# tnwei/waternet

Measured on NVIDIA H100. Metric: images/sec at 1080p batch16 (preprocess + gated-fusion forward, uint8 in -> uint8 out), higher is better.
Workload: dtype bf16 + fp8 corrections (v = hi + lo: hi x hi in bf16, both correction terms of the heavy layers as one e4m3 MMA; fp32 accumulate; 3-term bf16 elsewhere)

## Files before the change

### waternet_b200/csrc/common.cuh

```cuda
#pragma once

#include <cuda_runtime.h>
#include <stdint.h>
#include <stdio.h>

#include "../../include/waternet_b200.h"
#include "tiling.cuh"

namespace wn {

void set_error(const char* fmt, ...);

inline size_t align256(size_t v) { return (v + 255) / 256 * 256; }

#define WN_CUDA(call)                                                                   \
  do {                                                                                  \
    cudaError_t err__ = (call);                                                         \
    if (err__ != cudaSuccess) {                                                         \
      wn::set_error("%s:%d: %s -> %s", __FILE__, __LINE__, #call, cudaGetErrorString(err__)); \
      return WN_E_CUDA;                                                                 \
    }                                                                                   \
  } while (0)

#define WN_LAUNCH_CHECK(h)   \
  do {                       \
    (h)->launches++;         \
    WN_CUDA(cudaGetLastError()); \
  } while (0)

struct Tables {
  uint16_t gtab[256];
  uint16_t ctab[3072];
  int16_t ytab[256];
  int16_t fytab[256];
  uint8_t igtab[4096];
  uint8_t gamma[256];
  float div255[256];
};

void build_tables_host(Tables* t);

struct LayerDesc {
  int cin, cout, ks;
};
static const LayerDesc kCmg[8] = {{12, 128, 7}, {128, 128, 5}, {128, 128, 3}, {128, 64, 1},
                                  {64, 64, 7},  {64, 64, 5},   {64, 64, 3},   {64, 3, 3}};
static const LayerDesc kRef[3] = {{6, 32, 7}, {32, 32, 5}, {32, 3, 3}};
constexpr int kNumConvs = 17;

struct SimtLayer {
  int cin, cout, cout_pad, ks;
  float* w;
  float* bias;
};

struct UmmaWeights;
struct UmmaBwd;
struct VggWeights;

enum TimingSlot {
  kSlotConv0 = 0,
  kSlotPack = 17,
  kSlotGate = 18,
  kSlotStats = 19,
  kSlotLuts = 20,
  kSlotApply = 21,
  kSlotPost = 22,
  kNumSlots = 23
};
enum FwdStack { kStackAll = 0, kStackCmg = 1, kStackRefiners = 2 };
struct Timing {
  static constexpr int kMax = 8192;
  bool on;
  int used, created;
  cudaEvent_t a[kMax], b[kMax];
  int slot[kMax];
};

}

struct wn_handle {
  int device;
  uint64_t launches;
  wn::Tables* d_tables;
  bool packed;
  wn::SimtLayer simt[wn::kNumConvs];
  wn::UmmaWeights* umma;
  int sm_count;
  wn::Timing* timing;
  wn::UmmaBwd* bwd;
  long long chunk_pixels;
  wn::VggWeights* vgg;
  bool train_bf16;
};

namespace wn {

struct TimedScope {
  Timing* t;
  int idx;
  cudaStream_t stream;
  TimedScope(wn_handle* h, int slot, cudaStream_t s) : t(h->timing), idx(-1), stream(s) {
    if (!t || !t->on || t->used >= Timing::kMax) return;
    idx = t->used;
    if (idx >= t->created) {
      if (cudaEventCreate(&t->a[idx]) != cudaSuccess || cudaEventCreate(&t->b[idx]) != cudaSuccess) {
        idx = -1;
        return;
      }
      t->created = idx + 1;
    }
    t->used++;
    t->slot[idx] = slot;
    cudaEventRecord(t->a[idx], stream);
  }
  ~TimedScope() {
    if (idx >= 0) cudaEventRecord(t->b[idx], stream);
  }
};

size_t preprocess_workspace_bytes(int n, int h, int w);
int preprocess_u8(wn_handle* h, const uint8_t* rgb, int n, int height, int width, float* x,
                  float* wb, float* he, float* gc, uint8_t* wb_u8, uint8_t* he_u8, uint8_t* gc_u8,
                  void* workspace, size_t workspace_bytes, cudaStream_t stream);
int postprocess_u8(wn_handle* h, const float* out_nchw, uint8_t* out_nhwc, int n, int height,
                   int width, cudaStream_t stream);
size_t white_balance_gray_workspace_bytes(int n, int h, int w);
int white_balance_gray_u8(wn_handle* h, const uint8_t* gray, uint8_t* out, int n, int height, int width,
                          void* workspace, size_t workspace_bytes, cudaStream_t stream);
int resize_u8(wn_handle* h, const uint8_t* const* src, const int* src_h, const int* src_w, int n, uint8_t* dst,
              int dst_h, int dst_w, int swap_rb, cudaStream_t stream);
int preprocess_u8_planes(wn_handle* h, const uint8_t* rgb, int n, int height, int width, uint4* planes,
                         void* workspace, size_t workspace_bytes, cudaStream_t stream);
int preprocess_u8_luts(wn_handle* h, const uint8_t* rgb, int n, int height, int width, void* workspace,
                       size_t workspace_bytes, cudaStream_t stream);
int preprocess_u8_window_planes(wn_handle* h, const uint8_t* rgb, int n, const TileGeom& tiles, long long win0,
                                int count, uint4* planes, void* workspace, cudaStream_t stream);
struct RaggedImage {
  const uint8_t* rgb;
  int H, W;
  int th, tw, clip;
  int rows_per_slab, slabs;
  float lut_scale;
};
static_assert(sizeof(RaggedImage) == 40, "RaggedImage: engine.RAGGED_IMAGE_BYTES restates this size");
RaggedImage ragged_image(const uint8_t* rgb, int height, int width);
int preprocess_u8_ragged_luts(wn_handle* h, int n, const RaggedImage* imgs, int max_slabs, void* workspace,
                              cudaStream_t stream);
int preprocess_u8_ragged_planes(wn_handle* h, int n, const RaggedImage* imgs, const RaggedWindow* wins, int count,
                                int slot_h, int slot_w, uint4* planes, void* workspace, cudaStream_t stream);

int simt_pack_weights(wn_handle* h, const float* const* params, cudaStream_t stream);
void simt_free(wn_handle* h);
size_t simt_forward_workspace_bytes(int n, int h, int w);
int simt_forward(wn_handle* h, const float* const in[4], const int64_t in_strides[4][4], float* out,
                 int n, int height, int width, void* workspace, size_t workspace_bytes,
                 cudaStream_t stream, int stack = 0, int which = 0);

int simt_debug_layer(wn_handle* h, const float* const in[4], const int64_t in_strides[4][4], int n,
                     int height, int width, int layer, float* dst, void* workspace,
                     size_t workspace_bytes, cudaStream_t stream);

struct FwdBuffers {
  uint4* act0;
  uint4* a[8];
  uint4* r[3];
  float* cm;
  float* refined;
  int* exact_flag;
};
struct PeerOut {
  uint8_t* p[WN_MAX_PEERS];
  int n;
};
constexpr int kSchemeBf16 = 2;
inline int train_scheme(const wn_handle* h) { return h->train_bf16 ? kSchemeBf16 : 0; }
struct FwdOpts {
  int scheme = 0;
  int dbg_layer = -1;
  float* dbg_dst = nullptr;
  bool packed = false;
  bool hi_only = false;
  const int* run_if = nullptr;
  uint8_t* out_u8 = nullptr;
  PeerOut peers = {};
  int stack = kStackAll;
  bool refiner_l1 = false;
  const TileGeom* tiles = nullptr;
  long long win0 = 0;
  const RaggedWindow* rwin = nullptr;
};
int umma_forward_layers(wn_handle* h, const float* const in[4], const int64_t st[4][4], float* out, int n,
                        int height, int width, const FwdBuffers& b, cudaStream_t stream,
                        const FwdOpts& opts = FwdOpts());
int umma_debug_layer(wn_handle* h, const float* const in[4], const int64_t in_strides[4][4], int n,
                     int height, int width, int layer, float* dst, void* workspace,
                     size_t workspace_bytes, cudaStream_t stream, int scheme = 0);
int decode_planes(wn_handle* h, const uint4* src, float* dst, int planes_half, int n, int hw, cudaStream_t stream);
int umma_pack_weights(wn_handle* h, const float* const* params, cudaStream_t stream);
void umma_free(wn_handle* h);
size_t umma_forward_workspace_bytes(int n, int h, int w);
int umma_chunk_images(const wn_handle* h, int n, int height, int width);
int umma_forward(wn_handle* h, const float* const in[4], const int64_t in_strides[4][4], float* out,
                 int n, int height, int width, void* workspace, size_t workspace_bytes,
                 cudaStream_t stream, int scheme = 0, int stack = kStackAll, float* refined = nullptr);
size_t umma_forward_tiled_workspace_bytes(int n, int h, int w, int tile_h, int tile_w, long long max_pass_pixels,
                                          bool submodule);
int umma_forward_tiled(wn_handle* h, const float* const in[4], const int64_t in_strides[4][4], float* out, int n,
                       int height, int width, int tile_h, int tile_w, long long max_pass_pixels, void* workspace,
                       size_t workspace_bytes, cudaStream_t stream, int scheme, int stack = kStackAll, int which = 0);
size_t umma_enhance_workspace_bytes(int n, int h, int w);
int mirror_u8(wn_handle* h, const uint8_t* src, const PeerOut& peers, size_t bytes, const int* run_if, cudaStream_t stream);
int umma_enhance_u8(wn_handle* h, const uint8_t* rgb, uint8_t* out_u8, float* out_f32, int n, int height,
                    int width, void* workspace, size_t workspace_bytes, cudaStream_t stream, int scheme,
                    const PeerOut& peers = PeerOut());
size_t umma_enhance_tiled_workspace_bytes(int n, int h, int w, int tile_h, int tile_w, long long max_pass_pixels);
int umma_enhance_u8_tiled(wn_handle* h, const uint8_t* rgb, uint8_t* out_u8, float* out_f32, int n, int height,
                          int width, int tile_h, int tile_w, long long max_pass_pixels, void* workspace,
                          size_t workspace_bytes, cudaStream_t stream, int scheme);
size_t umma_enhance_ragged_workspace_bytes(const int* hs, const int* ws, int n, int tile_h, int tile_w,
                                           long long max_pass_pixels);
int umma_enhance_u8_ragged(wn_handle* h, const wn_ragged_image* images, int n, int tile_h, int tile_w,
                           long long max_pass_pixels, void* workspace, size_t workspace_bytes, cudaStream_t stream,
                           int scheme);
int umma_f8_overflowed(const wn_handle* h);

struct PackInArgs {
  const float* p[4];
  long long s[4][4];
};
inline PackInArgs pack_args(const float* const in[4], const int64_t st[4][4]) {
  PackInArgs pa;
  for (int t = 0; t < 4; t++) {
    pa.p[t] = in[t];
    for (int k = 0; k < 4; k++) pa.s[t][k] = st[t][k];
  }
  return pa;
}
int pack_inputs(wn_handle* h, const GridGeom& geo, const PackInArgs& in, int count, uint4* act0, int* flag,
                cudaStream_t stream, bool hi = false);
int pack_inputs(wn_handle* h, const TableGeom& geo, const PackInArgs* imgs, int count, uint4* act0, int* flag,
                cudaStream_t stream, bool hi = false);
size_t umma_forward_ragged_workspace_bytes(const int* hs, const int* ws, int n, int tile_h, int tile_w,
                                           long long max_pass_pixels);
int umma_forward_ragged(wn_handle* h, const wn_ragged_tensors* images, int n, int tile_h, int tile_w,
                        long long max_pass_pixels, void* workspace, size_t workspace_bytes, cudaStream_t stream,
                        int scheme);

constexpr long long kTrainMaxPixels = 8ll << 20;
constexpr long long kTiledTrainPassPixels = 2ll << 20;
int bwd_pack_weights(wn_handle* h, const float* const* params, cudaStream_t stream);
void bwd_free(wn_handle* h);
size_t train_workspace_bytes_padded(int n, int h, int w);
int forward_train(wn_handle* h, const float* const in[4], const int64_t in_strides[4][4], float* out, int n,
                  int height, int width, void* workspace, size_t workspace_bytes, cudaStream_t stream);
int backward(wn_handle* h, const float* grad_out, float* const* grads, float* const* input_grads, int n,
             int height, int width, void* workspace, size_t workspace_bytes, cudaStream_t stream);
size_t submodule_train_workspace_bytes(int n, int height, int width, int stack);
int confidence_maps_train(wn_handle* h, const float* const in[4], const int64_t in_strides[4][4], float* out_maps,
                          int n, int height, int width, void* workspace, size_t workspace_bytes, cudaStream_t stream);
int confidence_maps_backward(wn_handle* h, const float* grad_maps, float* const* grads, float* const* input_grads,
                             int n, int height, int width, void* workspace, size_t workspace_bytes,
                             cudaStream_t stream);
int refine_train(wn_handle* h, int which, const float* const in[4], const int64_t in_strides[4][4], float* out, int n,
                 int height, int width, void* workspace, size_t workspace_bytes, cudaStream_t stream);
int refine_backward(wn_handle* h, int which, const float* grad_out, float* const* grads, float* const* input_grads,
                    int n, int height, int width, void* workspace, size_t workspace_bytes, cudaStream_t stream);
int debug_backward_layer(wn_handle* h, int stack, int which, int buffer, const float* grad_out, float* const* grads,
                         int n, int height, int width, float* dst, void* workspace, size_t workspace_bytes,
                         cudaStream_t stream);
size_t backward_tiled_workspace_bytes(int n, int height, int width, int tile_h, int tile_w, long long max_pass_pixels);
int backward_tiled(wn_handle* h, const float* const in[4], const int64_t in_strides[4][4], const float* grad_out,
                   float* const* grads, float* const* input_grads, int n, int height, int width, int tile_h, int tile_w,
                   long long max_pass_pixels, void* workspace, size_t workspace_bytes, cudaStream_t stream);
size_t submodule_backward_tiled_workspace_bytes(int n, int height, int width, int tile_h, int tile_w,
                                                long long max_pass_pixels, int stack);
int submodule_backward_tiled(wn_handle* h, int stack, int which, const float* const in[4],
                             const int64_t in_strides[4][4], const float* grad, float* const* grads,
                             float* const* input_grads, int n, int height, int width, int tile_h, int tile_w,
                             long long max_pass_pixels, void* workspace, size_t workspace_bytes, cudaStream_t stream);
size_t train_ragged_workspace_bytes(const int* hs, const int* ws, int n);
int forward_train_ragged(wn_handle* h, const wn_ragged_tensors* images, int n, void* workspace, size_t workspace_bytes,
                         cudaStream_t stream);
int backward_ragged(wn_handle* h, const int* hs, const int* ws, const float* const* grad_out, float* const* grads,
                    float* const* input_grads, int n, void* workspace, size_t workspace_bytes, cudaStream_t stream);
size_t backward_ragged_tiled_workspace_bytes(const int* hs, const int* ws, int n, int tile_h, int tile_w,
                                             long long max_pass_pixels);
int backward_ragged_tiled(wn_handle* h, const wn_ragged_tensors* images, const float* const* grad_out,
                          float* const* grads, float* const* input_grads, int n, int tile_h, int tile_w,
                          long long max_pass_pixels, void* workspace, size_t workspace_bytes, cudaStream_t stream);

int vgg_pack_weights(wn_handle* h, const float* const* params, cudaStream_t stream);
void vgg_free(wn_handle* h);
size_t vgg_loss_workspace_bytes(int n, int height, int width, int tile_h, int tile_w, long long max_pass_pixels);
int vgg_perceptual_loss(wn_handle* h, const float* out, const int64_t out_strides[4], const float* ref,
                        const int64_t ref_strides[4], int n, int height, int width, int tile_h, int tile_w,
                        long long max_pass_pixels, float* loss, float* grad_out, void* workspace,
                        size_t workspace_bytes, cudaStream_t stream);
int vgg_debug_layer(wn_handle* h, const float* x, const int64_t strides[4], const float* ref,
                    const int64_t ref_strides[4], int n, int height, int width, int tile_h, int tile_w, int layer,
                    float* dst, void* workspace, size_t workspace_bytes, cudaStream_t stream);

}
```

### waternet_b200/csrc/conv_umma.cu

```cuda
#include "umma_conv.cuh"

namespace wn {

__device__ __forceinline__ bool pack_pixel(const PackInArgs& a, int n, int y, int x, float* v) {
  bool exact = true;
#pragma unroll
  for (int t = 0; t < 4; t++)
#pragma unroll
    for (int c = 0; c < 3; c++) {
      float f = __fmul_rn(a.p[t][n * a.s[t][0] + c * a.s[t][1] + y * a.s[t][2] + x * a.s[t][3]], 255.0f);
      float r = rintf(f);
      if (fabsf(f - r) <= 6.103515625e-5f && r >= 0.f && r <= 255.f) f = r; else exact = false;
      v[t * 3 + c] = f;
    }
  return exact;
}
template <bool HI>
__device__ __forceinline__ void store_packed(uint4* o, int hw, float* v) {
  v[12] = v[13] = v[14] = v[15] = 0.f;
  uint32_t hi[8], lo[8];
#pragma unroll
  for (int j = 0; j < 16; j += 2) {
    if constexpr (HI) {
      const __nv_bfloat162 hb = __floats2bfloat162_rn(v[j], v[j + 1]);
      hi[j >> 1] = *reinterpret_cast<const uint32_t*>(&hb);
      lo[j >> 1] = 0u;
    } else {
      split_bf16x2(v[j], v[j + 1], hi[j >> 1], lo[j >> 1]);
    }
  }
  o[0] = make_uint4(hi[0], hi[1], hi[2], hi[3]);
  o[hw] = make_uint4(hi[4], hi[5], hi[6], hi[7]);
  o[2 * (size_t)hw] = make_uint4(lo[0], lo[1], lo[2], lo[3]);
  o[3 * (size_t)hw] = make_uint4(lo[4], lo[5], lo[6], lo[7]);
}
__device__ __forceinline__ bool pack_slot_pixel(const PackInArgs& a, const SlotPixel& p, float* v) {
  return pack_pixel(a, p.img, p.y, p.x, v);
}
__device__ __forceinline__ bool pack_slot_pixel(const PackInArgs* __restrict__ imgs, const SlotPixel& p, float* v) {
  return pack_pixel(imgs[p.img], 0, p.y, p.x, v);
}

template <class Geom, class In, bool PLANES, bool FLAG, bool HI = false>
__global__ void __launch_bounds__(256)
pack_inputs_kernel(Geom geo, In in, uint4* __restrict__ out, int* __restrict__ exact_flag) {
  const int pix = blockIdx.x * 256 + threadIdx.x;
  const int hw = geo.slot_hw();
  bool exact = true;
  if (pix < hw) {
    const SlotPixel p = geo.at(blockIdx.y, pix);
    float v[16];
#pragma unroll
    for (int j = 0; j < 12; j++) v[j] = 0.f;
    if (p.valid) exact = pack_slot_pixel(in, p, v);
    if constexpr (PLANES) store_packed<HI>(out + (size_t)blockIdx.y * 4 * hw + pix, hw, v);
  }
  if constexpr (FLAG)
    if (!__syncthreads_and(exact) && threadIdx.x == 0) atomicExch(exact_flag, 0);
}

template <bool PLANES, bool FLAG, class Geom, class In>
static int launch_pack(wn_handle* h, const Geom& geo, const In& in, int count, uint4* act0, int* flag, bool reset,
                       cudaStream_t stream, bool hi = false) {
  TimedScope ts(h, kSlotPack, stream);
  if (reset) WN_CUDA(cudaMemsetAsync(flag, 1, sizeof(int), stream));
  const dim3 grid((unsigned)(((size_t)geo.slot_hw() + 255) / 256), count);
  if (PLANES && hi)
    pack_inputs_kernel<Geom, In, PLANES, FLAG, true><<<grid, 256, 0, stream>>>(geo, in, act0, flag);
  else
    pack_inputs_kernel<Geom, In, PLANES, FLAG><<<grid, 256, 0, stream>>>(geo, in, act0, flag);
  WN_LAUNCH_CHECK(h);
  return WN_OK;
}
int pack_inputs(wn_handle* h, const GridGeom& geo, const PackInArgs& in, int count, uint4* act0, int* flag,
                cudaStream_t stream, bool hi) {
  if (!act0) return launch_pack<false, true>(h, geo, in, count, nullptr, flag, true, stream);
  if (flag) return launch_pack<true, true>(h, geo, in, count, act0, flag, true, stream, hi);
  return launch_pack<true, false>(h, geo, in, count, act0, nullptr, false, stream, hi);
}
int pack_inputs(wn_handle* h, const TableGeom& geo, const PackInArgs* imgs, int count, uint4* act0, int* flag,
                cudaStream_t stream, bool hi) {
  if (!act0) return launch_pack<false, true>(h, geo, imgs, count, nullptr, flag, false, stream);
  return launch_pack<true, false>(h, geo, imgs, count, act0, nullptr, false, stream, hi);
}

__global__ void __launch_bounds__(256) store_kept_kernel(const float* __restrict__ src, int cs, int c0, int c,
                                                         float* __restrict__ dst, GridGeom geo) {
  const int pix = blockIdx.x * 256 + threadIdx.x;
  const int hw = geo.slot_hw();
  if (pix >= hw) return;
  const SlotPixel p = geo.at(blockIdx.y, pix);
  if (!p.kept) return;
  const float* s = src + ((size_t)blockIdx.y * cs + c0) * hw + pix;
  float* d = dst + (size_t)p.img * c * p.ihw + p.o;
  for (int k = 0; k < c; k++) d[k * p.ihw] = s[(size_t)k * hw];
}

enum UmmaLayer {
  kL1 = 0,
  kC2, kC3, kC4, kC5, kC6, kC7,
  kC8,
  kR2,
  kR3,
  kRL1,
  kNumUmmaLayers
};
struct UmmaLayerSpec {
  int ks, cinpad, npad, epi, concat, nblk, tps, slot;
  bool f8;
  int mw, ng, wgs;
};
static constexpr UmmaLayerSpec kSpecs[kNumUmmaLayers] = {
    {7, 16, 224, kEpiAct, 0, 1, 1, 0, false, 1, 1, 2},
    {5, 128, 128, kEpiAct, 0, 1, 5, 1, true, 1, 1, 2},
    {3, 128, 128, kEpiAct, 0, 1, 3, 2, true, 1, 1, 3},
    {1, 128, 64, kEpiAct, 1, 1, 1, 3, false, 1, 1, 3},
    {7, 64, 64, kEpiAct, 1, 1, 7, 4, true, 2, 1, 2},
    {5, 64, 64, kEpiAct, 1, 1, 5, 5, true, 2, 1, 2},
    {3, 64, 64, kEpiAct, 1, 1, 9, 6, true, 2, 1, 2},
    {3, 64, 16, kEpiSigmoid, 1, 1, 9, 7, false, 1, 1, 3},
    {5, 96, 32, kEpiAct, 1, 3, 5, 9, true, 1, 1, 3},
    {3, 96, 16, kEpiGate, 1, 1, 9, 10, false, 1, 1, 3},
    {7, 16, 96, kEpiAct, 0, 1, 1, 8, false, 1, 1, 3}};
#ifdef WN_UMMA_WGS2
static constexpr int layer_wgs(int) { return 2; }
#else
static constexpr int layer_wgs(int li) { return kSpecs[li].wgs; }
#endif

static_assert(kSpecs[kC2].f8 == kSpecs[kR2].f8, "L1 writes one format for both of its consumers");
static constexpr bool writes_f8(int li) { return li < kR3 && li != kC8 && kSpecs[li + 1].f8; }

static __global__ void __launch_bounds__(256)
mirror_u8_kernel(const uint8_t* __restrict__ src, PeerOut peers, size_t bytes, const int* __restrict__ run_if) {
  if (run_if && *run_if == 0) return;
  const size_t stride = (size_t)gridDim.x * blockDim.x, i0 = (size_t)blockIdx.x * blockDim.x + threadIdx.x;
#pragma unroll
  for (int k = 0; k < WN_MAX_PEERS; k++) {
    if (k >= peers.n) continue;
    uint8_t* dst = peers.p[k];
    const size_t vecs = (((reinterpret_cast<uintptr_t>(src) | reinterpret_cast<uintptr_t>(dst)) & 15) == 0) ? bytes / 16 : 0;
    for (size_t i = i0; i < vecs; i += stride) reinterpret_cast<uint4*>(dst)[i] = reinterpret_cast<const uint4*>(src)[i];
    for (size_t i = vecs * 16 + i0; i < bytes; i += stride) dst[i] = src[i];
  }
}
int mirror_u8(wn_handle* h, const uint8_t* src, const PeerOut& peers, size_t bytes, const int* run_if, cudaStream_t stream) {
  if (peers.n <= 0 || bytes == 0) return WN_OK;
  mirror_u8_kernel<<<4 * h->sm_count, 256, 0, stream>>>(src, peers, bytes, run_if);
  WN_LAUNCH_CHECK(h);
  return WN_OK;
}

struct UmmaWeights {
  uint8_t* stages8[kNumUmmaLayers];
  float* scale8[kNumUmmaLayers];
  int* overflow_dev;
  int* overflow_host;
  uint8_t* stages[kNumUmmaLayers];
  float* bias[kNumUmmaLayers];
  float* dense;
};

static size_t stage_bytes_total(const UmmaLayerSpec& s) { return (size_t)(s.cinpad / 16) * s.ks * s.ks * s.npad * 64; }

int umma_pack_weights(wn_handle* h, const float* const* params, cudaStream_t stream) {
  if (!h->umma) h->umma = (UmmaWeights*)calloc(1, sizeof(UmmaWeights));
  for (int i = 0; i < kNumUmmaLayers; i++) {
    if (!h->umma->stages[i]) WN_CUDA(cudaMalloc(&h->umma->stages[i], stage_bytes_total(kSpecs[i])));
    if (!h->umma->bias[i]) WN_CUDA(cudaMalloc(&h->umma->bias[i], kSpecs[i].npad * kSpecs[i].nblk * sizeof(float)));
    if (kSpecs[i].f8) {
      if (!h->umma->stages8[i]) WN_CUDA(cudaMalloc(&h->umma->stages8[i], stage_bytes_total(kSpecs[i])));
      if (!h->umma->scale8[i]) WN_CUDA(cudaMalloc(&h->umma->scale8[i], 4 * sizeof(float)));
    }
  }
  if (!h->umma->dense) WN_CUDA(cudaMalloc(&h->umma->dense, (size_t)224 * 128 * 49 * sizeof(float)));
  if (!h->umma->overflow_dev) WN_CUDA(cudaMalloc(&h->umma->overflow_dev, sizeof(int)));
  if (!h->umma->overflow_host) WN_CUDA(cudaHostAlloc(&h->umma->overflow_host, sizeof(int), cudaHostAllocDefault));
  UmmaWeights* u = h->umma;
  *u->overflow_host = 0;
  WN_CUDA(cudaMemsetAsync(u->overflow_dev, 0, sizeof(int), stream));
  auto W = [&](int conv) { return params[2 * conv]; };
  auto B = [&](int conv) { return params[2 * conv + 1]; };
  for (int li = 0; li < kNumUmmaLayers; li++) {
    const UmmaLayerSpec& s = kSpecs[li];
    const int kk = s.ks * s.ks;
    const int rows = s.npad * s.nblk;
    WN_CUDA(cudaMemsetAsync(u->dense, 0, (size_t)rows * s.cinpad * kk * sizeof(float), stream));
    WN_CUDA(cudaMemsetAsync(u->bias[li], 0, rows * sizeof(float), stream));
    auto scatter = [&](int conv, int co, int ci, int row_off, int split, int base0, int base1) -> int {
      scatter_weights_kernel<<<128, 256, 0, stream>>>(W(conv), u->dense, co, ci, kk, s.cinpad, row_off, split,
                                                      base0, base1, li == kL1 || li == kRL1 ? 255.0f : 1.0f);
      WN_LAUNCH_CHECK(h);
      scatter_bias_kernel<<<1, 256, 0, stream>>>(B(conv), u->bias[li], co, row_off);
      WN_LAUNCH_CHECK(h);
      return WN_OK;
    };
    int rc = WN_OK;
    if (li == kL1) {
      rc = scatter(0, 128, 12, 0, 12, 0, 0);
      for (int r = 0; r < 3 && !rc; r++)
        rc = scatter(8 + 3 * r, 32, 6, 128 + 32 * r, 3, 0, 3 * (r + 1));
    } else if (li >= kC2 && li <= kC8) {
      const int conv = li;
      const LayerDesc& d = kCmg[conv];
      rc = scatter(conv, d.cout, d.cin, 0, d.cin, 0, 0);
    } else if (li == kR2) {
      for (int r = 0; r < 3 && !rc; r++) rc = scatter(8 + 3 * r + 1, 32, 32, 32 * r, 32, 32 * r, 0);
    } else if (li == kRL1) {
      for (int r = 0; r < 3 && !rc; r++) rc = scatter(8 + 3 * r, 32, 6, 32 * r, 3, 0, 3 * (r + 1));
    } else {
      for (int r = 0; r < 3 && !rc; r++) rc = scatter(8 + 3 * r + 2, 3, 32, 3 * r, 32, 32 * r, 0);
    }
    if (rc) return rc;
    const int gw = s.npad / s.ng;
    const size_t group_bytes = stage_bytes_total(s) / s.ng;
    for (int g = 0; g < s.ng; g++) {
      pack_stages_kernel<<<256, 256, 0, stream>>>(u->dense, (__nv_bfloat16*)(u->stages[li] + g * group_bytes), gw,
                                                  s.cinpad, kk, s.concat, s.nblk, g * gw);
      WN_LAUNCH_CHECK(h);
    }
    if (s.f8) {
      WN_CUDA(cudaMemsetAsync(u->scale8[li], 0, 4 * sizeof(float), stream));
      f8_absmax_kernel<<<64, 256, 0, stream>>>(u->dense, (size_t)rows * s.cinpad * kk, u->scale8[li]);
      WN_LAUNCH_CHECK(h);
      f8_scale_finish_kernel<<<1, 1, 0, stream>>>(u->scale8[li]);
      WN_LAUNCH_CHECK(h);
      for (int g = 0; g < s.ng; g++) {
        pack_stages_f8_kernel<<<256, 256, 0, stream>>>(u->dense, u->stages8[li] + g * group_bytes, u->scale8[li], gw,
                                                       s.cinpad, kk, s.nblk, g * gw);
        WN_LAUNCH_CHECK(h);
      }
    }
  }
  return WN_OK;
}

void umma_free(wn_handle* h) {
  if (!h->umma) return;
  for (int i = 0; i < kNumUmmaLayers; i++) {
    if (h->umma->stages[i]) cudaFree(h->umma->stages[i]);
    if (h->umma->bias[i]) cudaFree(h->umma->bias[i]);
    if (h->umma->stages8[i]) cudaFree(h->umma->stages8[i]);
    if (h->umma->scale8[i]) cudaFree(h->umma->scale8[i]);
  }
  if (h->umma->dense) cudaFree(h->umma->dense);
  if (h->umma->overflow_dev) cudaFree(h->umma->overflow_dev);
  if (h->umma->overflow_host) cudaFreeHost(h->umma->overflow_host);
  free(h->umma);
  h->umma = nullptr;
}

static constexpr size_t kUmmaBytesPerPixel = 64 + 512 + 512 + 384 + 384 + 12;

static constexpr long long kDefaultChunkPixels = 8ll << 20;
static int umma_chunk(long long cap, int n, int h, int w) {
  if (cap <= 0 || cap > kDefaultChunkPixels) cap = kDefaultChunkPixels;
  long long per = (long long)h * w;
  long long nb = cap / (per > 0 ? per : 1);
  if (nb < 1) nb = 1;
  return nb < n ? (int)nb : n;
}
int umma_chunk_images(const wn_handle* h, int n, int height, int width) {
  return umma_chunk(h ? h->chunk_pixels : 0, n, height, width);
}

size_t umma_forward_workspace_bytes(int n, int h, int w) {
  const size_t nb = (size_t)umma_chunk(0, n, h, w);
  return nb * h * w * kUmmaBytesPerPixel + nb * h * 64 + 4096;
}

template <int LI, bool RAG>
static int launch_layer_as(wn_handle* h, int scheme, void* in_base, ConvArgs a, cudaStream_t stream) {
  constexpr UmmaLayerSpec s = kSpecs[LI];
  constexpr bool R = RAG && s.epi != kEpiSigmoid;
  const UmmaWeights* u = h->umma;
  constexpr int GW = s.npad / s.ng;
  if (scheme == kSchemeBf16)
    return launch_conv<s.ks, s.cinpad, GW, s.epi, s.concat, s.nblk, s.tps, kFmtHi, R, s.mw, s.ng, layer_wgs(LI)>(
        h, s.slot, u->stages[LI], u->bias[LI], in_base, a, stream);
  if (scheme == 1) {
    constexpr int FMT = (s.f8 ? kFmtIn8 : 0) | (writes_f8(LI) ? kFmtOut8 : 0);
    if constexpr ((FMT & kFmtOut8) != 0) a.f8_overflow = u->overflow_dev;
    if constexpr (s.f8) a.f8_scale = u->scale8[LI] + 1;
    return launch_conv<s.ks, s.cinpad, GW, s.epi, (s.f8 ? 0 : s.concat), s.nblk, s.tps, FMT, R, s.mw, s.ng,
                       layer_wgs(LI)>(h, s.slot, s.f8 ? u->stages8[LI] : u->stages[LI], u->bias[LI], in_base, a, stream);
  }
  return launch_conv<s.ks, s.cinpad, GW, s.epi, s.concat, s.nblk, s.tps, 0, R, s.mw, s.ng, layer_wgs(LI)>(
      h, s.slot, u->stages[LI], u->bias[LI], in_base, a, stream);
}
template <int LI>
static int launch_layer(wn_handle* h, int scheme, void* in_base, ConvArgs a, cudaStream_t stream) {
  return a.rwin ? launch_layer_as<LI, true>(h, scheme, in_base, a, stream)
                : launch_layer_as<LI, false>(h, scheme, in_base, a, stream);
}

__global__ void decode_planes_kernel(const uint4* __restrict__ src, float* __restrict__ dst, int planes_half, int hw,
                                     int f8) {
  const int n = blockIdx.z, plane = blockIdx.y;
  const int pix = blockIdx.x * blockDim.x + threadIdx.x;
  if (pix >= hw) return;
  const uint4 h4 = src[((size_t)n * 2 * planes_half + plane) * hw + pix];
  if (f8) {
    const uint4 l4 = src[((size_t)n * 2 * planes_half + planes_half + 2 * (plane >> 1)) * hw + pix];
    const uint32_t hs[4] = {h4.x, h4.y, h4.z, h4.w}, ls[4] = {l4.x, l4.y, l4.z, l4.w};
#pragma unroll
    for (int j = 0; j < 8; j++) {
      const float hi = __uint_as_float(((hs[j >> 1] >> ((j & 1) * 16)) & 0xffffu) << 16);
      const int byte = (plane & 1) * 8 + j;
      const uint32_t b8 = (ls[byte >> 2] >> ((byte & 3) * 8)) & 0xffu;
      const int e = (int)((b8 >> 3) & 15), m = (int)(b8 & 7);
      const float mag = e == 0 ? ldexpf((float)m, -9) : ldexpf((float)(8 + m), e - 10);
      const float lo = ((b8 & 0x80u) ? -mag : mag) * (1.f / 512.f);
      dst[((size_t)n * planes_half * 8 + plane * 8 + j) * hw + pix] = hi + lo;
    }
    return;
  }
  const uint4 l4 = src[((size_t)n * 2 * planes_half + planes_half + plane) * hw + pix];
  const uint32_t hs[4] = {h4.x, h4.y, h4.z, h4.w}, ls[4] = {l4.x, l4.y, l4.z, l4.w};
#pragma unroll
  for (int j = 0; j < 8; j++) {
    float hi = __uint_as_float(((hs[j >> 1] >> ((j & 1) * 16)) & 0xffffu) << 16);
    float lo = __uint_as_float(((ls[j >> 1] >> ((j & 1) * 16)) & 0xffffu) << 16);
    dst[((size_t)n * planes_half * 8 + plane * 8 + j) * hw + pix] = hi + lo;
  }
}

int decode_planes(wn_handle* h, const uint4* src, float* dst, int planes_half, int n, int hw, cudaStream_t stream) {
  decode_planes_kernel<<<dim3((hw + 255) / 256, planes_half, n), 256, 0, stream>>>(src, dst, planes_half, hw, 0);
  WN_LAUNCH_CHECK(h);
  return WN_OK;
}

int umma_forward_layers(wn_handle* h, const float* const in[4], const int64_t st[4][4], float* out, int n, int H,
                        int W, const FwdBuffers& b, cudaStream_t stream, const FwdOpts& o) {
  const int dbg_layer = o.dbg_layer;
  float* const dbg_dst = o.dbg_dst;
  if (!o.packed) {
    const int rc = pack_inputs(h, whole_images(H, W), pack_args(in, st), n, b.act0, b.exact_flag, stream,
                               o.scheme == kSchemeBf16);
    if (rc) return rc;
  }
  ConvArgs a;
  memset(&a, 0, sizeof(a));
  a.N = n; a.H = H; a.W = W;
  a.run_if = o.run_if;
  a.rwin = o.rwin;
  int rc;
  const bool f8 = o.scheme == 1;
  const int sc = o.scheme;
  auto dump = [&](int li) -> bool {
    const bool second = li == kL1 && dbg_layer == 8;
    if (dbg_layer != kSpecs[li].slot && !second) return false;
    const ActDst& d = second ? a.dst1 : a.dst0;
    decode_planes_kernel<<<dim3((H * W + 255) / 256, d.planes_half, n), 256, 0, stream>>>(d.base, dbg_dst, d.planes_half,
                                                                                      H * W, f8 && writes_f8(li));
    h->launches++;
    return true;
  };
  auto act = [&](uint4* d0, int c0, uint4* d1, int c1) {
    a.dst0.base = d0; a.dst0.planes_half = c0 / 8;
    a.dst1.base = d1; a.dst1.planes_half = c1 / 8;
    a.split_c = c0; a.cout = c0 + c1;
  };
  auto last = [&]() {
    a.out_f32 = out;
    a.out_u8 = o.out_u8;
    a.cm = o.stack == kStackRefiners ? nullptr : b.cm;
    a.refined_out = b.refined;
    if (o.tiles) {
      a.tiled = 1;
      a.tiles = *o.tiles;
      a.win0 = o.win0;
    }
  };
  const bool want_cmg = o.stack != kStackRefiners, want_ref = o.stack != kStackCmg;
  a.skip_lo = b.exact_flag;
  a.a_hi_only = o.hi_only ? 1 : 0;
  if (o.refiner_l1) {
    constexpr UmmaLayerSpec s = kSpecs[kRL1];
    act(b.r[1], 96, nullptr, 0);
    if (sc == kSchemeBf16)
      rc = launch_conv<s.ks, s.cinpad, s.npad, s.epi, s.concat, s.nblk, s.tps, kFmtHi, false, s.mw, s.ng,
                       layer_wgs(kRL1)>(h, s.slot, h->umma->stages[kRL1], h->umma->bias[kRL1], b.act0, a, stream);
    else
      rc = launch_conv<s.ks, s.cinpad, s.npad, s.epi, s.concat, s.nblk, s.tps, 0, false, s.mw, s.ng, layer_wgs(kRL1)>(
          h, s.slot, h->umma->stages[kRL1], h->umma->bias[kRL1], b.act0, a, stream);
    if (rc) return rc;
  } else {
    act(b.a[1], 128, b.r[1], b.r[1] ? 96 : 0);
    if ((rc = launch_layer<kL1>(h, sc, b.act0, a, stream))) return rc;
  }
  a.skip_lo = nullptr;
  a.a_hi_only = 0;
  if (dump(kL1)) return WN_OK;
  if (want_cmg) {
    act(b.a[2], 128, nullptr, 0);
    if ((rc = launch_layer<kC2>(h, sc, b.a[1], a, stream))) return rc;
    if (dump(kC2)) return WN_OK;
    act(b.a[3], 128, nullptr, 0);
    if ((rc = launch_layer<kC3>(h, sc, b.a[2], a, stream))) return rc;
    if (dump(kC3)) return WN_OK;
    act(b.a[4], 64, nullptr, 0);
    if ((rc = launch_layer<kC4>(h, sc, b.a[3], a, stream))) return rc;
    if (dump(kC4)) return WN_OK;
    act(b.a[5], 64, nullptr, 0);
    if ((rc = launch_layer<kC5>(h, sc, b.a[4], a, stream))) return rc;
    if (dump(kC5)) return WN_OK;
    act(b.a[6], 64, nullptr, 0);
    if ((rc = launch_layer<kC6>(h, sc, b.a[5], a, stream))) return rc;
    if (dump(kC6)) return WN_OK;
    act(b.a[7], 64, nullptr, 0);
    if ((rc = launch_layer<kC7>(h, sc, b.a[6], a, stream))) return rc;
    if (dump(kC7)) return WN_OK;
    const bool dump_maps = dbg_layer == kSpecs[kC8].slot;
    a.out_f32 = dump_maps ? dbg_dst : b.cm;
    if ((rc = launch_layer<kC8>(h, sc, b.a[7], a, stream))) return rc;
    if (dump_maps) return WN_OK;
  }
  if (!want_ref) return WN_OK;
  act(b.r[2], 96, nullptr, 0);
  if ((rc = launch_layer<kR2>(h, sc, b.r[1], a, stream))) return rc;
  if (dump(kR2)) return WN_OK;
  last();
  const bool dump_refined = dbg_layer == kSpecs[kR3].slot;
  if (dump_refined) {
    a.out_f32 = nullptr;
    a.out_u8 = nullptr;
    a.cm = nullptr;
    a.refined_out = dbg_dst;
  }
  if ((rc = launch_layer<kR3>(h, sc, b.r[2], a, stream))) return rc;
  if (dump_refined) return WN_OK;
  return o.out_u8 ? mirror_u8(h, o.out_u8, o.peers, (size_t)n * H * W * 3, o.run_if, stream) : WN_OK;
}

static FwdBuffers carve(void* workspace, int n, int H, int W) {
  const size_t px = (size_t)n * H * W;
  uint8_t* ws = (uint8_t*)(((uintptr_t)workspace + 1023) / 1024 * 1024);
  uint4* cmgAB[2];
  uint4* refAB[2];
  FwdBuffers b;
  memset(&b, 0, sizeof(b));
  b.act0 = (uint4*)ws;     ws += px * 64;
  cmgAB[0] = (uint4*)ws;   ws += px * 512;
  cmgAB[1] = (uint4*)ws;   ws += px * 512;
  refAB[0] = (uint4*)ws;   ws += px * 384;
  refAB[1] = (uint4*)ws;   ws += px * 384;
  b.cm = (float*)ws;       ws += px * 12;
  b.exact_flag = (int*)align256((uintptr_t)ws);
  for (int l = 1; l <= 7; l++) b.a[l] = cmgAB[(l - 1) & 1];
  b.r[1] = refAB[0];
  b.r[2] = refAB[1];
  return b;
}

static int umma_pass(wn_handle* h, const float* const in[4], const int64_t st[4][4], float* out, int n, int H, int W,
                     const FwdBuffers& b, cudaStream_t stream, FwdOpts o) {
  int rc = umma_forward_layers(h, in, st, out, n, H, W, b, stream, o);
  if (rc || o.scheme != 1 || o.dbg_layer >= 0) return rc;
  o.scheme = 0;
  o.packed = true;
  o.run_if = h->umma->overflow_dev;
  Timing* timing = h->timing;
  h->timing = nullptr;
  rc = umma_forward_layers(h, in, st, out, n, H, W, b, stream, o);
  h->timing = timing;
  return rc;
}

int umma_debug_layer(wn_handle* h, const float* const in[4], const int64_t in_strides[4][4], int n, int H, int W,
                     int layer, float* dst, void* workspace, size_t workspace_bytes, cudaStream_t stream, int scheme) {
  if (!h->umma || umma_chunk(0, n, H, W) != n || workspace_bytes < umma_forward_workspace_bytes(n, H, W)) {
    set_error("debug layer dump: weights not packed, batch too large for one pass or workspace too small");
    return WN_E_WORKSPACE;
  }
  int rc = get_encoder();
  if (rc) return rc;
  FwdOpts o;
  o.scheme = scheme;
  o.dbg_layer = layer;
  o.dbg_dst = dst;
  return umma_forward_layers(h, in, in_strides, nullptr, n, H, W, carve(workspace, n, H, W), stream, o);
}

static int effective_scheme(wn_handle* h, int scheme) {
  return (scheme == 1 && *h->umma->overflow_host) ? 0 : scheme;
}
static int mirror_overflow(wn_handle* h, int scheme, cudaStream_t stream) {
  if (scheme == 1)
    WN_CUDA(cudaMemcpyAsync(h->umma->overflow_host, h->umma->overflow_dev, sizeof(int), cudaMemcpyDeviceToHost, stream));
  return WN_OK;
}

int umma_forward(wn_handle* h, const float* const in[4], const int64_t in_strides[4][4], float* out, int n, int H,
                 int W, void* workspace, size_t workspace_bytes, cudaStream_t stream, int scheme, int stack,
                 float* refined) {
  if (!h->umma) {
    set_error("tensor-core weights have not been packed");
    return WN_E_STATE;
  }
  if (workspace_bytes < umma_forward_workspace_bytes(n, H, W)) {
    set_error("forward workspace too small: %zu < %zu", workspace_bytes, umma_forward_workspace_bytes(n, H, W));
    return WN_E_WORKSPACE;
  }
  int rc = get_encoder();
  if (rc) return rc;
  scheme = effective_scheme(h, scheme);
  const int nb = umma_chunk(h->chunk_pixels, n, H, W);
  for (int n0 = 0; n0 < n; n0 += nb) {
    const int cur = n - n0 < nb ? n - n0 : nb;
    const float* sub[4];
    for (int t = 0; t < 4; t++) sub[t] = in[t] + (long long)n0 * in_strides[t][0];
    FwdBuffers b = carve(workspace, cur, H, W);
    FwdOpts o;
    o.scheme = scheme;
    o.stack = stack;
      float* dst = out + (size_t)n0 * 3 * H * W;
    if (stack == kStackCmg) b.cm = dst;
    if (stack == kStackRefiners) { b.refined = refined + (size_t)n0 * 9 * H * W; dst = nullptr; }
    rc = umma_pass(h, sub, in_strides, dst, cur, H, W, b, stream, o);
    if (rc) return rc;
  }
  return mirror_overflow(h, scheme, stream);
}

size_t umma_enhance_workspace_bytes(int n, int h, int w) {
  const int nb = umma_chunk(0, n, h, w);
  return umma_forward_workspace_bytes(n, h, w) + align256(preprocess_workspace_bytes(nb, h, w)) + 1024;
}

int umma_enhance_u8(wn_handle* h, const uint8_t* rgb, uint8_t* out_u8, float* out_f32, int n, int H, int W,
                    void* workspace, size_t workspace_bytes, cudaStream_t stream, int scheme, const PeerOut& peers) {
  if (!h->umma) {
    set_error("tensor-core weights have not been packed");
    return WN_E_STATE;
  }
  if (workspace_bytes < umma_enhance_workspace_bytes(n, H, W)) {
    set_error("enhance workspace too small: %zu < %zu", workspace_bytes, umma_enhance_workspace_bytes(n, H, W));
    return WN_E_WORKSPACE;
  }
  int rc = get_encoder();
  if (rc) return rc;
  scheme = effective_scheme(h, scheme);
  const int nb = umma_chunk(h->chunk_pixels, n, H, W);
  uint8_t* pre_ws = (uint8_t*)align256((uintptr_t)workspace);
  const size_t pre_b = align256(preprocess_workspace_bytes(nb, H, W));
  void* fwd_ws = pre_ws + pre_b;
  const int64_t none[4][4] = {};
  const float* no_in[4] = {nullptr, nullptr, nullptr, nullptr};
  for (int n0 = 0; n0 < n; n0 += nb) {
    const int cur = n - n0 < nb ? n - n0 : nb;
    FwdBuffers b = carve(fwd_ws, cur, H, W);
    WN_CUDA(cudaMemsetAsync(b.exact_flag, 1, sizeof(int), stream));
    rc = preprocess_u8_planes(h, rgb + (size_t)n0 * H * W * 3, cur, H, W, b.act0, pre_ws, pre_b, stream);
    if (rc) return rc;
    FwdOpts o;
    o.scheme = scheme;
    o.packed = true;
    o.hi_only = true;
    o.out_u8 = out_u8 + (size_t)n0 * H * W * 3;
    o.peers.n = peers.n;
    for (int k = 0; k < peers.n; k++) o.peers.p[k] = peers.p[k] + (size_t)n0 * H * W * 3;
    rc = umma_pass(h, no_in, none, out_f32 ? out_f32 + (size_t)n0 * 3 * H * W : nullptr, cur, H, W, b, stream, o);
    if (rc) return rc;
  }
  return mirror_overflow(h, scheme, stream);
}

size_t umma_enhance_tiled_workspace_bytes(int n, int h, int w, int tile_h, int tile_w, long long max_pass_pixels) {
  if (n <= 0 || h <= 0 || w <= 0 || tile_h <= 0 || tile_w <= 0 || max_pass_pixels < 0) return 0;
  if ((size_t)h * w > (size_t)0x7fffffff / 3 || n > 65535) return 0;
  const TileGeom g = tile_geom(h, w, tile_h, tile_w);
  const long long p = tile_pass_windows(g, n, max_pass_pixels ? max_pass_pixels : kDefaultChunkPixels);
  return (size_t)p * g.win_h * g.win_w * kUmmaBytesPerPixel + 4096 + align256(preprocess_workspace_bytes(n, h, w)) +
         1024;
}

int umma_enhance_u8_tiled(wn_handle* h, const uint8_t* rgb, uint8_t* out_u8, float* out_f32, int n, int H, int W,
                          int tile_h, int tile_w, long long max_pass_pixels, void* workspace, size_t workspace_bytes,
                          cudaStream_t stream, int scheme) {
  if (!h->umma) {
    set_error("tensor-core weights have not been packed");
    return WN_E_STATE;
  }
  const size_t need = umma_enhance_tiled_workspace_bytes(n, H, W, tile_h, tile_w, max_pass_pixels);
  if (workspace_bytes < need) {
    set_error("tiled enhance workspace too small: %zu < %zu", workspace_bytes, need);
    return WN_E_WORKSPACE;
  }
  int rc = get_encoder();
  if (rc) return rc;
  scheme = effective_scheme(h, scheme);
  const TileGeom g = tile_geom(H, W, tile_h, tile_w);
  const long long total = (long long)n * g.ny * g.nx;
  const long long per_pass = tile_pass_windows(g, n, max_pass_pixels ? max_pass_pixels : kDefaultChunkPixels);
  uint8_t* pre_ws = (uint8_t*)align256((uintptr_t)workspace);
  const size_t pre_b = align256(preprocess_workspace_bytes(n, H, W));
  void* fwd_ws = pre_ws + pre_b;
  if ((rc = preprocess_u8_luts(h, rgb, n, H, W, pre_ws, pre_b, stream))) return rc;
  const int64_t none[4][4] = {};
  const float* no_in[4] = {nullptr, nullptr, nullptr, nullptr};
  for (long long w0 = 0; w0 < total; w0 += per_pass) {
    const int cur = (int)(total - w0 < per_pass ? total - w0 : per_pass);
    FwdBuffers b = carve(fwd_ws, cur, g.win_h, g.win_w);
    WN_CUDA(cudaMemsetAsync(b.exact_flag, 1, sizeof(int), stream));
    rc = preprocess_u8_window_planes(h, rgb, n, g, w0, cur, b.act0, pre_ws, stream);
    if (rc) return rc;
    FwdOpts o;
    o.scheme = scheme;
    o.packed = true;
    o.hi_only = true;
    o.out_u8 = out_u8;
    o.tiles = &g;
    o.win0 = w0;
    rc = umma_pass(h, no_in, none, out_f32, cur, g.win_h, g.win_w, b, stream, o);
    if (rc) return rc;
  }
  return mirror_overflow(h, scheme, stream);
}

static size_t ragged_table_bytes(int n, size_t windows) {
  return align256(align256((size_t)n * sizeof(RaggedImage)) + windows * sizeof(RaggedWindow));
}
static long long ragged_pass_pixels(long long max_pass_pixels) {
  return max_pass_pixels ? max_pass_pixels : kDefaultChunkPixels;
}
static size_t ragged_workspace(int n, const std::vector<RaggedWindow>& wins, const std::vector<RaggedPass>& passes) {
  return (size_t)largest_pass_pixels(passes) * kUmmaBytesPerPixel + 4096 +
         align256(preprocess_workspace_bytes(n, 1, 1)) + ragged_table_bytes(n, wins.size()) + 1024;
}

size_t umma_enhance_ragged_workspace_bytes(const int* hs, const int* ws, int n, int tile_h, int tile_w,
                                           long long max_pass_pixels) {
  std::vector<RaggedWindow> wins;
  std::vector<RaggedPass> passes;
  ragged_plan(hs, ws, n, tile_h, tile_w, ragged_pass_pixels(max_pass_pixels), &wins, &passes);
  return ragged_workspace(n, wins, passes);
}

int umma_enhance_u8_ragged(wn_handle* h, const wn_ragged_image* images, int n, int tile_h, int tile_w,
                           long long max_pass_pixels, void* workspace, size_t workspace_bytes, cudaStream_t stream,
                           int scheme) {
  if (!h->umma) {
    set_error("tensor-core weights have not been packed");
    return WN_E_STATE;
  }
  std::vector<int> hs(n), ws(n);
  for (int i = 0; i < n; i++) {
    hs[i] = images[i].height;
    ws[i] = images[i].width;
  }
  std::vector<RaggedWindow> wins;
  std::vector<RaggedPass> passes;
  ragged_plan(hs.data(), ws.data(), n, tile_h, tile_w, ragged_pass_pixels(max_pass_pixels), &wins, &passes);
  const size_t need = ragged_workspace(n, wins, passes);
  if (workspace_bytes < need) {
    set_error("ragged enhance workspace too small: %zu < %zu", workspace_bytes, need);
    return WN_E_WORKSPACE;
  }
  int rc = get_encoder();
  if (rc) return rc;
  scheme = effective_scheme(h, scheme);
  uint8_t* pre_ws = (uint8_t*)align256((uintptr_t)workspace);
  const size_t pre_b = align256(preprocess_workspace_bytes(n, 1, 1));
  uint8_t* table = pre_ws + pre_b;
  const size_t img_b = align256((size_t)n * sizeof(RaggedImage));
  void* fwd_ws = table + ragged_table_bytes(n, wins.size());
  std::vector<uint8_t> host(img_b + wins.size() * sizeof(RaggedWindow));
  RaggedImage* imgs = reinterpret_cast<RaggedImage*>(host.data());
  int max_slabs = 1;
  for (int i = 0; i < n; i++) {
    imgs[i] = ragged_image(images[i].rgb, images[i].height, images[i].width);
    max_slabs = imgs[i].slabs > max_slabs ? imgs[i].slabs : max_slabs;
  }
  for (RaggedWindow& w : wins) {
    w.rgb = images[w.img].rgb;
    w.out_u8 = images[w.img].out_u8;
    w.out_f32 = images[w.img].out_f32;
  }
  memcpy(host.data() + img_b, wins.data(), wins.size() * sizeof(RaggedWindow));
  WN_CUDA(cudaMemcpyAsync(table, host.data(), host.size(), cudaMemcpyHostToDevice, stream));
  const RaggedImage* d_imgs = reinterpret_cast<const RaggedImage*>(table);
  const RaggedWindow* d_wins = reinterpret_cast<const RaggedWindow*>(table + img_b);
  if ((rc = preprocess_u8_ragged_luts(h, n, d_imgs, max_slabs, pre_ws, stream))) return rc;
  const int64_t none[4][4] = {};
  const float* no_in[4] = {nullptr, nullptr, nullptr, nullptr};
  for (const RaggedPass& p : passes) {
    FwdBuffers b = carve(fwd_ws, p.count, p.slot_h, p.slot_w);
    WN_CUDA(cudaMemsetAsync(b.exact_flag, 1, sizeof(int), stream));
    rc = preprocess_u8_ragged_planes(h, n, d_imgs, d_wins + p.first, p.count, p.slot_h, p.slot_w, b.act0, pre_ws,
                                     stream);
    if (rc) return rc;
    FwdOpts o;
    o.scheme = scheme;
    o.packed = true;
    o.hi_only = true;
    o.rwin = d_wins + p.first;
    rc = umma_pass(h, no_in, none, nullptr, p.count, p.slot_h, p.slot_w, b, stream, o);
    if (rc) return rc;
  }
  return mirror_overflow(h, scheme, stream);
}

size_t umma_forward_tiled_workspace_bytes(int n, int h, int w, int tile_h, int tile_w, long long max_pass_pixels,
                                          bool submodule) {
  const TileGeom g = tile_geom(h, w, tile_h, tile_w);
  const size_t px = (size_t)tile_pass_windows(g, n, max_pass_pixels ? max_pass_pixels : kDefaultChunkPixels) *
                    g.win_h * g.win_w;
  return px * kUmmaBytesPerPixel + 4096 + 256 + (submodule ? align256(px * 9 * sizeof(float)) + 256 : 0);
}

int umma_forward_tiled(wn_handle* h, const float* const in[4], const int64_t in_strides[4][4], float* out, int n,
                       int H, int W, int tile_h, int tile_w, long long max_pass_pixels, void* workspace,
                       size_t workspace_bytes, cudaStream_t stream, int scheme, int stack, int which) {
  if (!h->umma) {
    set_error("tensor-core weights have not been packed");
    return WN_E_STATE;
  }
  const bool sub = stack != kStackAll;
  const size_t need = umma_forward_tiled_workspace_bytes(n, H, W, tile_h, tile_w, max_pass_pixels, sub);
  if (workspace_bytes < need) {
    set_error("tiled forward workspace too small: %zu < %zu", workspace_bytes, need);
    return WN_E_WORKSPACE;
  }
  int rc = get_encoder();
  if (rc) return rc;
  scheme = effective_scheme(h, scheme);
  const TileGeom g = tile_geom(H, W, tile_h, tile_w);
  const long long total = (long long)n * g.ny * g.nx;
  const long long per_pass = tile_pass_windows(g, n, max_pass_pixels ? max_pass_pixels : kDefaultChunkPixels);
  const size_t win_px = (size_t)g.win_h * g.win_w;
  uint8_t* base = (uint8_t*)align256((uintptr_t)workspace);
  int* exact = (int*)base;
  float* refined = (float*)(base + 256);
  void* fwd_ws = base + 256 + (sub ? align256(per_pass * win_px * 9 * sizeof(float)) : 0);
  const PackInArgs pa = pack_args(in, in_strides);
  if ((rc = pack_inputs(h, whole_images(H, W), pa, n, nullptr, exact, stream))) return rc;
  for (long long w0 = 0; w0 < total; w0 += per_pass) {
    const int cur = (int)(total - w0 < per_pass ? total - w0 : per_pass);
    const GridGeom geo = {g, w0};
    FwdBuffers b = carve(fwd_ws, cur, g.win_h, g.win_w);
    b.exact_flag = exact;
    if ((rc = pack_inputs(h, geo, pa, cur, b.act0, nullptr, stream))) return rc;
    FwdOpts o;
    o.scheme = scheme;
    o.packed = true;
    o.stack = stack;
    if (stack == kStackRefiners) b.refined = refined;
    if (!sub) {
      o.tiles = &g;
      o.win0 = w0;
    }
    rc = umma_pass(h, in, in_strides, sub ? nullptr : out, cur, g.win_h, g.win_w, b, stream, o);
    if (rc) return rc;
    if (sub) {
      TimedScope ts(h, kSlotGate, stream);
      const bool maps = stack == kStackCmg;
      store_kept_kernel<<<dim3((unsigned)((win_px + 255) / 256), cur), 256, 0, stream>>>(
          maps ? b.cm : refined, maps ? 3 : 9, maps ? 0 : 3 * which, 3, out, geo);
      WN_LAUNCH_CHECK(h);
    }
  }
  return mirror_overflow(h, scheme, stream);
}

static size_t ragged_fp32_table_bytes(int n, size_t windows) {
  return align256(align256((size_t)n * sizeof(PackInArgs)) + windows * sizeof(RaggedWindow));
}
static size_t ragged_fp32_workspace(int n, const std::vector<RaggedWindow>& wins,
                                    const std::vector<RaggedPass>& passes) {
  return (size_t)largest_pass_pixels(passes) * kUmmaBytesPerPixel + 4096 + 256 +
         ragged_fp32_table_bytes(n, wins.size()) + 1024;
}

size_t umma_forward_ragged_workspace_bytes(const int* hs, const int* ws, int n, int tile_h, int tile_w,
                                           long long max_pass_pixels) {
  std::vector<RaggedWindow> wins;
  std::vector<RaggedPass> passes;
  ragged_plan(hs, ws, n, tile_h, tile_w, ragged_pass_pixels(max_pass_pixels), &wins, &passes);
  return ragged_fp32_workspace(n, wins, passes);
}

int umma_forward_ragged(wn_handle* h, const wn_ragged_tensors* images, int n, int tile_h, int tile_w,
                        long long max_pass_pixels, void* workspace, size_t workspace_bytes, cudaStream_t stream,
                        int scheme) {
  if (!h->umma) {
    set_error("tensor-core weights have not been packed");
    return WN_E_STATE;
  }
  std::vector<int> hs(n), ws(n);
  for (int i = 0; i < n; i++) {
    hs[i] = images[i].height;
    ws[i] = images[i].width;
  }
  std::vector<RaggedWindow> wins;
  std::vector<RaggedPass> passes;
  ragged_plan(hs.data(), ws.data(), n, tile_h, tile_w, ragged_pass_pixels(max_pass_pixels), &wins, &passes);
  const size_t need = ragged_fp32_workspace(n, wins, passes);
  if (workspace_bytes < need) {
    set_error("ragged forward workspace too small: %zu < %zu", workspace_bytes, need);
    return WN_E_WORKSPACE;
  }
  int rc = get_encoder();
  if (rc) return rc;
  scheme = effective_scheme(h, scheme);
  uint8_t* base = (uint8_t*)align256((uintptr_t)workspace);
  int* exact = (int*)base;
  uint8_t* table = base + 256;
  const size_t img_b = align256((size_t)n * sizeof(PackInArgs));
  void* fwd_ws = table + ragged_fp32_table_bytes(n, wins.size());
  std::vector<uint8_t> host(img_b + wins.size() * sizeof(RaggedWindow));
  PackInArgs* imgs = reinterpret_cast<PackInArgs*>(host.data());
  for (int i = 0; i < n; i++) {
    const wn_ragged_tensors& t = images[i];
    const float* in[4] = {t.x, t.wb, t.he, t.gc};
    imgs[i] = pack_args(in, t.in_strides);
  }
  for (RaggedWindow& w : wins) w.out_f32 = images[w.img].out;
  memcpy(host.data() + img_b, wins.data(), wins.size() * sizeof(RaggedWindow));
  WN_CUDA(cudaMemcpyAsync(table, host.data(), host.size(), cudaMemcpyHostToDevice, stream));
  const PackInArgs* d_imgs = reinterpret_cast<const PackInArgs*>(table);
  TableGeom geo = {reinterpret_cast<const RaggedWindow*>(table + img_b), 0, 0, 0, tile_h, tile_w};
  WN_CUDA(cudaMemsetAsync(exact, 1, sizeof(int), stream));
  for (const RaggedPass& p : passes) {
    geo.set_pass(p);
    if ((rc = pack_inputs(h, geo, d_imgs, p.count, nullptr, exact, stream))) return rc;
  }
  const int64_t none[4][4] = {};
  const float* no_in[4] = {nullptr, nullptr, nullptr, nullptr};
  for (const RaggedPass& p : passes) {
    FwdBuffers b = carve(fwd_ws, p.count, p.slot_h, p.slot_w);
    b.exact_flag = exact;
    geo.set_pass(p);
    if ((rc = pack_inputs(h, geo, d_imgs, p.count, b.act0, nullptr, stream))) return rc;
    FwdOpts o;
    o.scheme = scheme;
    o.packed = true;
    o.rwin = geo.rwin();
    rc = umma_pass(h, no_in, none, nullptr, p.count, p.slot_h, p.slot_w, b, stream, o);
    if (rc) return rc;
  }
  return mirror_overflow(h, scheme, stream);
}

int umma_f8_overflowed(const wn_handle* h) { return h->umma && h->umma->overflow_host ? *h->umma->overflow_host : 0; }

}
```

### waternet_b200/csrc/umma_conv.cuh

```cuda
#pragma once

#include <cuda.h>
#include <cuda_bf16.h>

#include "common.cuh"
#include "wgmma_ops.cuh"

namespace wn {

__device__ __forceinline__ uint32_t smem_u32(const void* p) {
  return (uint32_t)__cvta_generic_to_shared(p);
}
__device__ __forceinline__ void mbar_init(uint64_t* bar, uint32_t count) {
  asm volatile("mbarrier.init.shared::cta.b64 [%0], %1;" ::"r"(smem_u32(bar)), "r"(count));
}
__device__ __forceinline__ void mbar_wait(uint64_t* bar, uint32_t parity) {
  for (uint32_t it = 0; it < (1u << 26); it++) {
    uint32_t done;
    asm volatile(
        "{\n\t.reg .pred p;\n\t"
        "mbarrier.try_wait.parity.shared::cta.b64 p, [%1], %2;\n\t"
        "selp.u32 %0, 1, 0, p;\n\t}"
        : "=r"(done)
        : "r"(smem_u32(bar)), "r"(parity)
        : "memory");
    if (done) return;
  }
  __trap();
}
__device__ __forceinline__ void mbar_arrive(uint64_t* bar) {
  asm volatile("mbarrier.arrive.shared::cta.b64 _, [%0];" ::"r"(smem_u32(bar)) : "memory");
}
__device__ __forceinline__ void mbar_expect_tx(uint64_t* bar, uint32_t bytes) {
  asm volatile("mbarrier.arrive.expect_tx.shared::cta.b64 _, [%0], %1;" ::"r"(smem_u32(bar)), "r"(bytes)
               : "memory");
}
__device__ __forceinline__ void tma_load_5d(void* dst, const CUtensorMap* tmap, uint64_t* bar, int c0,
                                            int c1, int c2, int c3, int c4) {
  asm volatile(
      "cp.async.bulk.tensor.5d.shared::cluster.global.mbarrier::complete_tx::bytes [%0], [%1, {%3, %4, %5, %6, %7}], [%2];"
      ::"r"(smem_u32(dst)), "l"(tmap), "r"(smem_u32(bar)), "r"(c0), "r"(c1), "r"(c2), "r"(c3), "r"(c4)
      : "memory");
}
__device__ __forceinline__ void bulk_load(void* dst, const void* src, uint32_t bytes, uint64_t* bar) {
  asm volatile(
      "cp.async.bulk.shared::cluster.global.mbarrier::complete_tx::bytes [%0], [%1], %2, [%3];" ::"r"(
          smem_u32(dst)),
      "l"(src), "r"(bytes), "r"(smem_u32(bar))
      : "memory");
}
__device__ __forceinline__ uint64_t make_desc(uint32_t addr, uint32_t lbo, uint32_t sbo) {
  return (uint64_t)((addr >> 4) & 0x3fff) | ((uint64_t)((lbo >> 4) & 0x3fff) << 16) |
         ((uint64_t)((sbo >> 4) & 0x3fff) << 32);
}
__device__ __forceinline__ void wg_fence() { asm volatile("wgmma.fence.sync.aligned;" ::: "memory"); }
__device__ __forceinline__ void wg_commit() { asm volatile("wgmma.commit_group.sync.aligned;" ::: "memory"); }
template <int PENDING>
__device__ __forceinline__ void wg_wait() { asm volatile("wgmma.wait_group.sync.aligned %0;" ::"n"(PENDING) : "memory"); }
__device__ __forceinline__ void wg_bar(int id) { asm volatile("bar.sync %0, 128;" ::"r"(id) : "memory"); }
__device__ __forceinline__ uint32_t pack_e4m3x4(float f0, float f1, float f2, float f3) {
  uint16_t lo, hi;
  asm("cvt.rn.satfinite.e4m3x2.f32 %0, %1, %2;" : "=h"(lo) : "f"(f1), "f"(f0));
  asm("cvt.rn.satfinite.e4m3x2.f32 %0, %1, %2;" : "=h"(hi) : "f"(f3), "f"(f2));
  return (uint32_t)lo | ((uint32_t)hi << 16);
}
__device__ __forceinline__ uint16_t pack_e4m3x2(float f0, float f1) {
  uint16_t v;
  asm("cvt.rn.satfinite.e4m3x2.f32 %0, %1, %2;" : "=h"(v) : "f"(f1), "f"(f0));
  return v;
}

enum Epilogue { kEpiAct = 0, kEpiSigmoid = 1, kEpiGate = 2, kEpiDgrad = 3 };

constexpr int kStageLd = 36;

constexpr int kFmtIn8 = 1, kFmtOut8 = 2, kFmtHi = 4;
constexpr int kWgs3ProducerRegs = 24, kWgs3ConsumerRegs = 160;
template <int KS, int CIN_PAD, int NPAD, int CONCAT = 0, int NBLK = 1, int TPS = 1, int FMT = 0, int MW = 1,
          int NG = 1, int WGS = 2>
struct UmmaCfg {
  static constexpr bool F8IN = (FMT & kFmtIn8) != 0;
  static constexpr bool HI = (FMT & kFmtHi) != 0;
  static constexpr bool DUAL = CONCAT != 0 && !HI;
  static constexpr int TILE_W = 8 * MW, TILE_H = 8 * WGS;
  static constexpr int CONSUMER_WARPS = 4 * WGS;
  static constexpr int WARP_A = CONSUMER_WARPS, WARP_B = CONSUMER_WARPS + 1;
  static constexpr int THREADS = WGS == 2 ? 320 : 512;
  static constexpr int HALO_W = TILE_W + KS - 1, HALO_H = TILE_H + KS - 1;
  static constexpr int NCHUNK = CIN_PAD / 16;
  static constexpr int PLANE_BYTES = HALO_W * HALO_H * 16;
  static constexpr int A_STAGE = (4 * PLANE_BYTES + 1023) / 1024 * 1024;
  static constexpr int B_TAP = NPAD * 64;
  static constexpr int B_STAGE = TPS * B_TAP;
  static_assert((KS * KS) % TPS == 0, "taps per weight stage must divide the filter");
  static constexpr int NSTAGE_PER_CHUNK = KS * KS / TPS;
  static constexpr int STAGING = WGS * 64 * kStageLd * 4;
  static constexpr int BIAS_BYTES = NG * NBLK * NPAD * 4;
  static constexpr int TAIL = 512 + (BIAS_BYTES > 1536 ? BIAS_BYTES : 1536);
  static constexpr int BUDGET = 227 * 1024 - 1024 - TAIL - STAGING;
  static constexpr int NA_WANT = NCHUNK == 1 ? 2 : KS == 1 ? 6 : 3;
  static constexpr int NB_FIT = (BUDGET - NA_WANT * A_STAGE) / B_STAGE;
  static constexpr int NB = NB_FIT > 8 ? 8 : NB_FIT < 2 ? 2 : NB_FIT;
  static constexpr int NA_FIT = (BUDGET - NB * B_STAGE) / A_STAGE;
  static constexpr int NA = NA_FIT > NA_WANT ? NA_WANT : NA_FIT;
  static_assert(!F8IN || !CONCAT, "fp8 corrections: the [hi | second part] weight layout");
  static_assert(!HI || FMT == kFmtHi, "single-pass bf16 reads and writes bf16 planes only");
  static constexpr int CPB = NCHUNK / NBLK;
  static constexpr int BLK_COLS = DUAL ? 2 * NPAD : NPAD;
  static constexpr int COLS = NBLK * BLK_COLS;
  static constexpr int ACC = COLS / 2;
  static constexpr int ACC8 = F8IN ? ACC : 1;
  static constexpr int SMEM_BYTES = NA * A_STAGE + NB * B_STAGE + STAGING + TAIL + 1024;
  static_assert(NA >= 1, "halo tile does not fit in shared memory");
  static_assert(NCHUNK % NBLK == 0, "chunks must split evenly over the diagonal blocks");
  static_assert(NPAD % 16 == 0 && (DUAL ? 2 : 1) * NPAD <= 256, "invalid wgmma N");
  static_assert(MW == 1 || MW == 2, "one or two m64 blocks per warpgroup");
  static_assert(WGS == 2 || (WGS == 3 && MW == 1), "two consumer warpgroups, or three of one m64 block each");
  static_assert(NG == 1 || NBLK == 1, "column groups of a block-diagonal layer");
  static_assert(MW * (ACC + (F8IN ? ACC8 : 0)) <= 128, "accumulators do not fit in registers");
  static constexpr size_t GROUP_BYTES = (size_t)NCHUNK * NSTAGE_PER_CHUNK * B_STAGE;
};

struct ActDst {
  uint4* base;
  int planes_half;
};

struct ConvArgs {
  const uint8_t* wpk;
  const float* bias;
  int N, H, W;
  int in_planes_half;
  int tiles_x, tiles_y;
  ActDst dst0, dst1;
  int split_c;
  int cout;
  float* out_f32;
  const float* cm;
  uint8_t* out_u8;
  const int* skip_lo;
  int a_hi_only;
  float* refined_out;
  const uint4* mask_base;
  int mask_planes_half;
  const float* f8_scale;
  int* f8_overflow;
  const int* run_if;
  int tiled;
  long long win0;
  TileGeom tiles;
  const RaggedWindow* rwin;
};

__device__ __forceinline__ uint32_t pack_bf16x2(__nv_bfloat16 a, __nv_bfloat16 b) {
  return (uint32_t)__bfloat16_as_ushort(a) | ((uint32_t)__bfloat16_as_ushort(b) << 16);
}
__device__ __forceinline__ void split_bf16x2(float f0, float f1, uint32_t& hi, uint32_t& lo) {
  const __nv_bfloat162 h = __floats2bfloat162_rn(f0, f1);
  hi = *reinterpret_cast<const uint32_t*>(&h);
  const float h0 = __uint_as_float(hi << 16), h1 = __uint_as_float(hi & 0xffff0000u);
  const __nv_bfloat162 l = __floats2bfloat162_rn(f0 - h0, f1 - h1);
  lo = *reinterpret_cast<const uint32_t*>(&l);
}

template <int EPI, bool OUT8, bool RAG = false, bool HI = false>
__device__ __forceinline__ void epilogue16(const ConvArgs& g, const float* s_bias, const float* f, int ch, int n,
                                           int gx, int gy, bool valid = true) {
  const size_t hw = (size_t)g.H * g.W;
  const size_t pix = (size_t)gy * g.W + gx;
  if constexpr (EPI == kEpiAct || EPI == kEpiDgrad) {
    if (ch >= g.cout) return;
    if constexpr (OUT8) {
      uint32_t hi[8], l8[4], h8[4];
      float vmax = 0.f;
#pragma unroll
      for (int j = 0; j < 16; j += 4) {
        float v[4], r[4];
#pragma unroll
        for (int t = 0; t < 4; t++) {
          v[t] = fmaxf(f[j + t] + s_bias[ch + j + t], 0.f);
          if constexpr (RAG) v[t] = valid ? v[t] : 0.f;
          vmax = fmaxf(vmax, v[t]);
        }
#pragma unroll
        for (int t = 0; t < 4; t += 2) {
          const __nv_bfloat162 h = __floats2bfloat162_rn(v[t], v[t + 1]);
          const uint32_t hb = *reinterpret_cast<const uint32_t*>(&h);
          hi[(j + t) >> 1] = hb;
          r[t] = (v[t] - __uint_as_float(hb << 16)) * 512.f;
          r[t + 1] = (v[t + 1] - __uint_as_float(hb & 0xffff0000u)) * 512.f;
        }
        l8[j >> 2] = pack_e4m3x4(r[0], r[1], r[2], r[3]);
        h8[j >> 2] = pack_e4m3x4(v[0], v[1], v[2], v[3]);
      }
      if (!(vmax <= 448.f) && g.f8_overflow) atomicOr(g.f8_overflow, 1);
      const bool second = ch >= g.split_c;
      const ActDst& d = second ? g.dst1 : g.dst0;
      const int chl = second ? ch - g.split_c : ch;
      uint4* p_hi = d.base + ((size_t)n * 2 * d.planes_half + (chl >> 3)) * hw + pix;
      uint4* p_f8 = d.base + ((size_t)n * 2 * d.planes_half + d.planes_half + 2 * (chl >> 4)) * hw + pix;
      p_hi[0] = make_uint4(hi[0], hi[1], hi[2], hi[3]);
      p_hi[hw] = make_uint4(hi[4], hi[5], hi[6], hi[7]);
      p_f8[0] = make_uint4(l8[0], l8[1], l8[2], l8[3]);
      p_f8[hw] = make_uint4(h8[0], h8[1], h8[2], h8[3]);
    } else {
#pragma unroll
      for (int q = 0; q < 16; q += 8) {
        const int c = ch + q;
        if (c >= g.cout) break;
        uint32_t hi[4], lo[4];
        uint32_t mask[4] = {0xffffffffu, 0xffffffffu, 0xffffffffu, 0xffffffffu};
        if constexpr (EPI == kEpiDgrad) {
          if (g.mask_base) {
            const uint4 m = g.mask_base[((size_t)n * 2 * g.mask_planes_half + (c >> 3)) * hw + pix];
            mask[0] = m.x; mask[1] = m.y; mask[2] = m.z; mask[3] = m.w;
          }
        }
#pragma unroll
        for (int j = 0; j < 8; j += 2) {
          float f0, f1;
          if constexpr (EPI == kEpiDgrad) {
            f0 = (mask[j >> 1] & 0x0000ffffu) ? f[q + j] : 0.f;
            f1 = (mask[j >> 1] & 0xffff0000u) ? f[q + j + 1] : 0.f;
          } else {
            f0 = fmaxf(f[q + j] + s_bias[c + j], 0.f);
            f1 = fmaxf(f[q + j + 1] + s_bias[c + j + 1], 0.f);
            if constexpr (RAG) {
              f0 = valid ? f0 : 0.f;
              f1 = valid ? f1 : 0.f;
            }
          }
          if constexpr (HI) {
            const __nv_bfloat162 hb = __floats2bfloat162_rn(f0, f1);
            hi[j >> 1] = *reinterpret_cast<const uint32_t*>(&hb);
            lo[j >> 1] = 0u;
          } else {
            split_bf16x2(f0, f1, hi[j >> 1], lo[j >> 1]);
          }
        }
        const bool second = c >= g.split_c;
        const ActDst& d = second ? g.dst1 : g.dst0;
        const int plane = (second ? c - g.split_c : c) >> 3;
        uint4* p_hi = d.base + ((size_t)n * 2 * d.planes_half + plane) * hw + pix;
        p_hi[0] = make_uint4(hi[0], hi[1], hi[2], hi[3]);
        p_hi[(size_t)d.planes_half * hw] = make_uint4(lo[0], lo[1], lo[2], lo[3]);
      }
    }
  } else {
    if (ch != 0) return;
    const size_t o = (size_t)n * 3 * hw + pix;
    if constexpr (EPI == kEpiSigmoid) {
#pragma unroll
      for (int c = 0; c < 3; c++) g.out_f32[o + c * hw] = 1.0f / (1.0f + expf(-(f[c] + s_bias[c])));
    } else {
      float r[9];
#pragma unroll
      for (int j = 0; j < 9; j++) r[j] = fmaxf(f[j] + s_bias[j], 0.f);
      if (g.refined_out) {
#pragma unroll
        for (int j = 0; j < 9; j++) g.refined_out[(size_t)n * 9 * hw + pix + j * hw] = r[j];
      }
      if (g.cm) {
        const float c0 = g.cm[o], c1 = g.cm[o + hw], c2 = g.cm[o + 2 * hw];
        float v[3];
#pragma unroll
        for (int c = 0; c < 3; c++)
          v[c] = __fadd_rn(__fadd_rn(__fmul_rn(r[c], c0), __fmul_rn(r[3 + c], c1)), __fmul_rn(r[6 + c], c2));
        size_t oo = o, ohw = hw, o8 = ((size_t)n * hw + pix) * 3;
        float* out_f32 = g.out_f32;
        uint8_t* out_u8 = g.out_u8;
        if constexpr (RAG) {
          const RaggedWindow& t = g.rwin[n];
          const int y = t.ys + gy, x = t.xs + gx;
          if (y < t.ky0 || y >= t.ky1 || x < t.kx0 || x >= t.kx1) return;
          ohw = (size_t)t.H * t.W;
          oo = (size_t)y * t.W + x;
          o8 = oo * 3;
          out_f32 = t.out_f32;
          out_u8 = t.out_u8;
        } else if (g.tiled) {
          const TileWindow t = tile_window(g.tiles, g.win0 + n);
          const int y = t.ys + gy, x = t.xs + gx;
          if (y < t.ky0 || y >= t.ky1 || x < t.kx0 || x >= t.kx1) return;
          ohw = (size_t)g.tiles.H * g.tiles.W;
          const size_t ipix = (size_t)y * g.tiles.W + x;
          oo = (size_t)t.img * 3 * ohw + ipix;
          o8 = ((size_t)t.img * ohw + ipix) * 3;
        }
        if (out_f32) {
#pragma unroll
          for (int c = 0; c < 3; c++) out_f32[oo + c * ohw] = v[c];
        }
        if (out_u8) {
          uint8_t* q = out_u8 + o8;
#pragma unroll
          for (int c = 0; c < 3; c++) q[c] = (uint8_t)(int)__fmul_rn(fminf(fmaxf(v[c], 0.0f), 1.0f), 255.0f);
        }
      }
    }
  }
}

template <int KS, int CIN_PAD, int NPAD, int EPI, int CONCAT, int NBLK, int TPS, int FMT = 0, bool RAG = false,
          int MW = 1, int NG = 1, int WGS = 2>
__global__ void __launch_bounds__(WGS == 2 ? 320 : 512, 1)
conv_umma_kernel(const __grid_constant__ CUtensorMap tmap_in, const ConvArgs g) {
  using C = UmmaCfg<KS, CIN_PAD, NPAD, CONCAT, NBLK, TPS, FMT, MW, NG, WGS>;
  constexpr bool F8IN = C::F8IN, DUAL = C::DUAL, OUT8 = (FMT & kFmtOut8) != 0;
  static_assert(!OUT8 || EPI == kEpiAct, "fp8 planes are written by the activation epilogue only");
  static_assert(!RAG || EPI == kEpiAct || EPI == kEpiGate, "ragged passes mask activations and store the gate");
  if (g.run_if != nullptr && *reinterpret_cast<const volatile int*>(g.run_if) == 0) return;
  extern __shared__ uint8_t smem_raw[];
  uint8_t* smem = reinterpret_cast<uint8_t*>((reinterpret_cast<uintptr_t>(smem_raw) + 1023) & ~(uintptr_t)1023);
  uint8_t* a_stages = smem;
  uint8_t* b_stages = smem + C::NA * C::A_STAGE;
  float* staging = reinterpret_cast<float*>(b_stages + C::NB * C::B_STAGE);
  uint8_t* tail = reinterpret_cast<uint8_t*>(staging) + C::STAGING;
  uint64_t* a_full = reinterpret_cast<uint64_t*>(tail);
  uint64_t* a_empty = a_full + C::NA;
  uint64_t* b_full = a_empty + C::NA;
  uint64_t* b_empty = b_full + C::NB;
  float* s_bias = reinterpret_cast<float*>(tail + 512);
  static_assert((2 * 6 + 2 * 8) * 8 <= 512 && C::BIAS_BYTES <= C::TAIL - 512, "barrier / bias area");

  const int tid = threadIdx.x, warp = tid >> 5, lane = tid & 31;
  const int num_tiles = g.tiles_x * g.tiles_y * g.N * NG;
  if (tid == 0) {
    for (int i = 0; i < C::NA; i++) { mbar_init(&a_full[i], 1); mbar_init(&a_empty[i], C::CONSUMER_WARPS); }
    for (int i = 0; i < C::NB; i++) { mbar_init(&b_full[i], 1); mbar_init(&b_empty[i], C::CONSUMER_WARPS); }
    asm volatile("fence.mbarrier_init.release.cluster;" ::: "memory");
  }
  for (int i = tid; i < NG * NBLK * NPAD; i += C::THREADS) s_bias[i] = g.bias[i];
  __syncthreads();
  if constexpr (WGS == 3) {
    if (warp >= C::CONSUMER_WARPS) {
      asm volatile("setmaxnreg.dec.sync.aligned.u32 %0;" ::"n"(kWgs3ProducerRegs));
      if (warp > C::WARP_B) return;
    }
  }
  if (warp == C::WARP_A) {
    if (lane == 0) {
      int stage = 0;
      uint32_t phase = 0;
      for (int tile = blockIdx.x; tile < num_tiles; tile += gridDim.x) {
        const int pt = tile / NG;
        const int n = pt / (g.tiles_x * g.tiles_y);
        const int rem = pt - n * g.tiles_x * g.tiles_y;
        const int ty = rem / g.tiles_x, tx = rem - ty * g.tiles_x;
        const int x0 = tx * C::TILE_W - KS / 2, y0 = ty * C::TILE_H - KS / 2;
        for (int c = 0; c < C::NCHUNK; c++) {
          mbar_wait(&a_empty[stage], phase ^ 1);
          uint8_t* dst = a_stages + stage * C::A_STAGE;
          mbar_expect_tx(&a_full[stage], (C::HI || g.a_hi_only ? 2 : 4) * C::PLANE_BYTES);
          tma_load_5d(dst, &tmap_in, &a_full[stage], 0, x0, y0, 2 * c, n);
          if (!C::HI && !g.a_hi_only)
            tma_load_5d(dst + 2 * C::PLANE_BYTES, &tmap_in, &a_full[stage], 0, x0, y0, g.in_planes_half + 2 * c, n);
          if (++stage == C::NA) { stage = 0; phase ^= 1; }
        }
      }
    }
    return;
  }
  if (warp == C::WARP_B) {
    if (lane == 0) {
      int stage = 0;
      uint32_t phase = 0;
      for (int tile = blockIdx.x; tile < num_tiles; tile += gridDim.x) {
        const uint8_t* wpk = g.wpk + (size_t)(tile % NG) * C::GROUP_BYTES;
        for (int it = 0; it < C::NCHUNK * C::NSTAGE_PER_CHUNK; it++) {
          mbar_wait(&b_empty[stage], phase ^ 1);
          mbar_expect_tx(&b_full[stage], C::B_STAGE);
          bulk_load(b_stages + stage * C::B_STAGE, wpk + (size_t)it * C::B_STAGE, C::B_STAGE, &b_full[stage]);
          if (++stage == C::NB) { stage = 0; phase ^= 1; }
        }
      }
    }
    return;
  }
  if constexpr (WGS == 3) asm volatile("setmaxnreg.inc.sync.aligned.u32 %0;" ::"n"(kWgs3ConsumerRegs));

  const int wg = warp >> 2, wtid = tid & 127;
  const bool skip_lo = (g.skip_lo != nullptr && *g.skip_lo != 0) || g.a_hi_only;
  const float dscale0 = F8IN && WGS == 2 ? *g.f8_scale : 1.f;
  constexpr uint32_t kSboA = C::HALO_W * 16;
  constexpr uint32_t kLboB = (CONCAT ? 2 * NPAD : NPAD) * 16;
  float acc[MW][C::ACC], acc8[MW][C::ACC8];
  int astage = 0, bstage = 0, pend_a = -1, pend_b = -1;
  uint32_t aphase = 0, bphase = 0;
  auto release = [&]() {
    if (lane == 0) {
      if (pend_b >= 0) mbar_arrive(&b_empty[pend_b]);
      if (pend_a >= 0) mbar_arrive(&a_empty[pend_a]);
    }
    pend_a = pend_b = -1;
  };
  for (int tile = blockIdx.x; tile < num_tiles; tile += gridDim.x) {
#pragma unroll
    for (int mb = 0; mb < MW; mb++) {
#pragma unroll
      for (int i = 0; i < C::ACC; i++) acc[mb][i] = 0.f;
#pragma unroll
      for (int i = 0; i < C::ACC8; i++) acc8[mb][i] = 0.f;
    }
#pragma unroll
    for (int c = 0; c < C::NCHUNK; c++) {
      mbar_wait(&a_full[astage], aphase);
      const uint32_t a_base = smem_u32(a_stages + astage * C::A_STAGE) + (uint32_t)(wg * 8 * C::HALO_W * 16);
      const int blk = NBLK > 1 ? c / C::CPB : 0;
      for (int tg = 0; tg < C::NSTAGE_PER_CHUNK; tg++) {
        mbar_wait(&b_full[bstage], bphase);
        const uint32_t b_base = smem_u32(b_stages + bstage * C::B_STAGE);
        wg_fence();
#pragma unroll
        for (int t = 0; t < TPS; t++) {
          const int tap = tg * TPS + t;
          const int ky = tap / KS, kx = tap - ky * KS;
          const uint32_t a_tap = a_base + (uint32_t)((ky * C::HALO_W + kx) * 16);
          const uint32_t b_tap = b_base + (uint32_t)(t * C::B_TAP);
          const uint64_t a_hi0 = make_desc(a_tap, C::PLANE_BYTES, kSboA);
#pragma unroll
          for (int mb = 0; mb < MW; mb++) {
            const uint64_t a_hi = a_hi0 + mb * (128 >> 4);
            const uint64_t a_lo = MW == 1 ? make_desc(a_tap + 2 * C::PLANE_BYTES, C::PLANE_BYTES, kSboA)
                                          : a_hi + ((2 * C::PLANE_BYTES) >> 4);
#pragma unroll
            for (int b = 0; b < NBLK; b++) {
              if (NBLK > 1 && b != blk) continue;
              float* d = acc[mb] + b * C::BLK_COLS / 2;
              if constexpr (C::HI) {
                wgmma_bf16<NPAD>(d, a_hi, make_desc(b_tap, kLboB, 128));
              } else if constexpr (F8IN) {
                wgmma_bf16<NPAD>(d, a_hi, make_desc(b_tap, NPAD * 16, 128));
                wgmma_e4m3<NPAD>(acc8[mb] + b * C::BLK_COLS / 2, a_lo, make_desc(b_tap + NPAD * 32, NPAD * 16, 128));
              } else if constexpr (CONCAT) {
                wgmma_bf16<2 * NPAD>(d, a_hi, make_desc(b_tap, kLboB, 128));
                if (!skip_lo) wgmma_bf16<NPAD>(d, a_lo, make_desc(b_tap, kLboB, 128));
              } else {
                wgmma_bf16<NPAD>(d, a_hi, make_desc(b_tap, kLboB, 128));
                if (!skip_lo) wgmma_bf16<NPAD>(d, a_lo, make_desc(b_tap, kLboB, 128));
                wgmma_bf16<NPAD>(d, a_hi, make_desc(b_tap + 2 * NPAD * 16, kLboB, 128));
              }
            }
          }
        }
        wg_commit();
        wg_wait<1>();
        release();
        pend_b = bstage;
        if (tg == C::NSTAGE_PER_CHUNK - 1) pend_a = astage;
        if (++bstage == C::NB) { bstage = 0; bphase ^= 1; }
      }
      if (++astage == C::NA) { astage = 0; aphase ^= 1; }
    }
    wg_wait<0>();
    release();

    const int pt = tile / NG, c0 = (tile % NG) * NPAD;
    const int n = pt / (g.tiles_x * g.tiles_y);
    const int rem = pt - n * g.tiles_x * g.tiles_y;
    const int ty = rem / g.tiles_x, tx = rem - ty * g.tiles_x;
    float* stg = staging + wg * 64 * kStageLd;
    const int frow = (warp & 3) * 16 + (lane >> 2), fcol = (lane & 3) * 2;
    const int r = wtid & 63, half = wtid >> 6;
    const int m = wg * 64 + r;
    const int gy = ty * C::TILE_H + (m >> 3);
    const float dscale = F8IN && WGS == 3 ? *g.f8_scale : dscale0;
    constexpr int NCH = NBLK * NPAD;
#pragma unroll
    for (int mb = 0; mb < MW; mb++) {
      const int gx = tx * C::TILE_W + mb * 8 + (m & 7);
      const bool inside = gx < g.W && gy < g.H;
      bool valid = true;
      if constexpr (RAG) valid = gx < g.rwin[n].vw && gy < g.rwin[n].vh;
#pragma unroll
      for (int ch0 = 0; ch0 < NCH; ch0 += 32) {
#pragma unroll
        for (int j = 0; j < 4; j++) {
          const int ch = ch0 + 8 * j;
          if (ch < NCH) {
            const int col = NBLK > 1 ? (ch / NPAD) * C::BLK_COLS + ch % NPAD : ch;
            float v[4];
#pragma unroll
            for (int k = 0; k < 4; k++) {
              v[k] = acc[mb][col / 2 + k];
              if constexpr (DUAL) v[k] += acc[mb][(col + NPAD) / 2 + k];
              if constexpr (F8IN) v[k] = (v[k] + acc8[mb][col / 2 + k]) * dscale;
            }
            float* s = stg + frow * kStageLd + 8 * j + fcol;
            *reinterpret_cast<float2*>(s) = make_float2(v[0], v[1]);
            *reinterpret_cast<float2*>(s + 8 * kStageLd) = make_float2(v[2], v[3]);
          }
        }
        wg_bar(1 + wg);
        const int cb = ch0 + 16 * half;
        if (cb < NCH && inside) {
          float f[16];
          const float4* s = reinterpret_cast<const float4*>(stg + r * kStageLd + 16 * half);
#pragma unroll
          for (int q = 0; q < 4; q++) {
            const float4 x = s[q];
            f[4 * q] = x.x; f[4 * q + 1] = x.y; f[4 * q + 2] = x.z; f[4 * q + 3] = x.w;
          }
          epilogue16<EPI, OUT8, RAG, C::HI>(g, s_bias, f, c0 + cb, n, gx, gy, valid);
        }
        wg_bar(1 + wg);
      }
    }
  }
}

static __global__ void scatter_weights_kernel(const float* __restrict__ src, float* __restrict__ dense, int co, int ci,
                                       int kk, int cinpad, int row_off, int split, int base0, int base1,
                                       float divisor) {
  const int total = co * ci * kk;
  for (int i = blockIdx.x * blockDim.x + threadIdx.x; i < total; i += gridDim.x * blockDim.x) {
    int t = i % kk;
    int c = (i / kk) % ci;
    int o = i / (kk * ci);
    int cd = c < split ? base0 + c : base1 + (c - split);
    dense[((size_t)(row_off + o) * cinpad + cd) * kk + t] = __fdiv_rn(src[i], divisor);
  }
}
static __global__ void scatter_bias_kernel(const float* __restrict__ src, float* __restrict__ dst, int co, int row_off) {
  for (int i = blockIdx.x * blockDim.x + threadIdx.x; i < co; i += gridDim.x * blockDim.x) dst[row_off + i] = src[i];
}
static __global__ void pack_stages_kernel(const float* __restrict__ dense, __nv_bfloat16* __restrict__ out, int npad,
                                   int cinpad, int kk, int concat, int nblk, int row_off = 0) {
  const int nchunk = cinpad / 16, cpb = nchunk / nblk;
  const size_t total = (size_t)nchunk * kk * 2 * 2 * npad * 8;
  for (size_t i = (size_t)blockIdx.x * blockDim.x + threadIdx.x; i < total; i += (size_t)gridDim.x * blockDim.x) {
    int e = (int)(i % 8);
    size_t r = i / 8;
    int k8, split, nrow;
    if (concat) {
      int row2 = (int)(r % (2 * npad)); r /= 2 * npad;
      k8 = (int)(r % 2); r /= 2;
      split = row2 >= npad;
      nrow = row2 - split * npad;
    } else {
      nrow = (int)(r % npad); r /= npad;
      k8 = (int)(r % 2); r /= 2;
      split = (int)(r % 2); r /= 2;
    }
    int tap = (int)(r % kk);
    int chunk = (int)(r / kk);
    int cin = chunk * 16 + k8 * 8 + e;
    int row = row_off + (chunk / cpb) * npad + nrow;
    float w = dense[((size_t)row * cinpad + cin) * kk + tap];
    __nv_bfloat16 hi = __float2bfloat16_rn(w);
    out[i] = split == 0 ? hi : __float2bfloat16_rn(w - __bfloat162float(hi));
  }
}


static __global__ void f8_absmax_kernel(const float* __restrict__ dense, size_t n, float* __restrict__ scale) {
  __shared__ float smax[256];
  float m = 0.f;
  for (size_t i = (size_t)blockIdx.x * blockDim.x + threadIdx.x; i < n; i += (size_t)gridDim.x * blockDim.x)
    m = fmaxf(m, fabsf(dense[i]));
  smax[threadIdx.x] = m;
  __syncthreads();
  for (int o = 128; o > 0; o >>= 1) {
    if ((int)threadIdx.x < o) smax[threadIdx.x] = fmaxf(smax[threadIdx.x], smax[threadIdx.x + o]);
    __syncthreads();
  }
  if (threadIdx.x == 0) atomicMax(reinterpret_cast<unsigned int*>(scale + 2), __float_as_uint(smax[0]));
}
static __global__ void f8_scale_finish_kernel(float* __restrict__ scale) {
  const float mx = fmaxf(scale[2], 1e-30f);
  const float ws = exp2f(floorf(log2f(224.f / mx)));
  scale[0] = ws;
  scale[1] = 1.f / (512.f * ws);
}
static __global__ void pack_stages_f8_kernel(const float* __restrict__ dense, uint8_t* __restrict__ out,
                                             const float* __restrict__ scale, int npad, int cinpad, int kk, int nblk,
                                             int row_off) {
  const int nchunk = cinpad / 16, cpb = nchunk / nblk, rows = npad;
  const size_t tap_bytes = (size_t)rows * 64;
  const float ws = scale[0];
  const size_t total = (size_t)nchunk * kk * rows * 8;
  for (size_t i = (size_t)blockIdx.x * blockDim.x + threadIdx.x; i < total; i += (size_t)gridDim.x * blockDim.x) {
    size_t r = i;
    const int cp = (int)(r % 8); r /= 8;
    const int row = (int)(r % rows); r /= rows;
    const int tap = (int)(r % kk);
    const int chunk = (int)(r / kk);
    const int wrow = row_off + (chunk / cpb) * npad + row;
    float w[2], wl[2];
    uint16_t hb[2];
#pragma unroll
    for (int t = 0; t < 2; t++) {
      w[t] = dense[((size_t)wrow * cinpad + chunk * 16 + 2 * cp + t) * kk + tap];
      const __nv_bfloat16 h = __float2bfloat16_rn(w[t]);
      hb[t] = __bfloat16_as_ushort(h);
      wl[t] = w[t] - __bfloat162float(h);
    }
    uint8_t* base = out + ((size_t)chunk * kk + tap) * tap_bytes;
    const int c = 2 * cp;
#pragma unroll
    for (int t = 0; t < 2; t++)
      hb[t] = __bfloat16_as_ushort(__float2bfloat16_rn(__bfloat162float(__ushort_as_bfloat16(hb[t])) * ws * 512.f));
    *reinterpret_cast<uint32_t*>(base + ((size_t)(c / 8) * rows + row) * 16 + (c % 8) * 2) =
        (uint32_t)hb[0] | ((uint32_t)hb[1] << 16);
    uint8_t* p1 = base + (size_t)rows * 32;
    *reinterpret_cast<uint16_t*>(p1 + ((size_t)0 * rows + row) * 16 + c) = pack_e4m3x2(w[0] * ws, w[1] * ws);
    *reinterpret_cast<uint16_t*>(p1 + ((size_t)1 * rows + row) * 16 + c) =
        pack_e4m3x2(wl[0] * ws * 512.f, wl[1] * ws * 512.f);
  }
}

typedef CUresult (*EncodeTiledFn)(CUtensorMap*, CUtensorMapDataType, cuuint32_t, void*, const cuuint64_t*,
                                  const cuuint64_t*, const cuuint32_t*, const cuuint32_t*, CUtensorMapInterleave,
                                  CUtensorMapSwizzle, CUtensorMapL2promotion, CUtensorMapFloatOOBfill);
static EncodeTiledFn g_encode = nullptr;

static int get_encoder() {
  if (g_encode) return WN_OK;
  cudaDriverEntryPointQueryResult q;
  void* fn = nullptr;
  WN_CUDA(cudaGetDriverEntryPoint("cuTensorMapEncodeTiled", &fn, cudaEnableDefault, &q));
  if (!fn || q != cudaDriverEntryPointSuccess) {
    set_error("cuTensorMapEncodeTiled is not available from this driver");
    return WN_E_UNSUPPORTED;
  }
  g_encode = (EncodeTiledFn)fn;
  return WN_OK;
}

static int make_tmap(CUtensorMap* tm, void* base, int planes_total, int N, int H, int W, int halo_w, int halo_h) {
  cuuint64_t dims[5] = {8, (cuuint64_t)W, (cuuint64_t)H, (cuuint64_t)planes_total, (cuuint64_t)N};
  cuuint64_t strides[4] = {16, (cuuint64_t)W * 16, (cuuint64_t)H * W * 16, (cuuint64_t)planes_total * H * W * 16};
  cuuint32_t box[5] = {8, (cuuint32_t)halo_w, (cuuint32_t)halo_h, 2, 1};
  cuuint32_t estr[5] = {1, 1, 1, 1, 1};
  CUresult r = g_encode(tm, CU_TENSOR_MAP_DATA_TYPE_BFLOAT16, 5, base, dims, strides, box, estr,
                        CU_TENSOR_MAP_INTERLEAVE_NONE, CU_TENSOR_MAP_SWIZZLE_NONE, CU_TENSOR_MAP_L2_PROMOTION_L2_128B,
                        CU_TENSOR_MAP_FLOAT_OOB_FILL_NONE);
  if (r != CUDA_SUCCESS) {
    set_error("cuTensorMapEncodeTiled failed with %d (planes=%d N=%d H=%d W=%d box=%dx%d)", (int)r, planes_total, N, H,
              W, halo_w, halo_h);
    return WN_E_CUDA;
  }
  return WN_OK;
}

template <int KS, int CIN_PAD, int NPAD, int EPI, int CONCAT = 0, int NBLK = 1, int TPS = 1, int FMT = 0,
          bool RAG = false, int MW = 1, int NG = 1, int WGS = 2>
static int launch_conv(wn_handle* h, int slot, const uint8_t* wpk, const float* bias, void* in_base, ConvArgs a,
                       cudaStream_t stream) {
  using C = UmmaCfg<KS, CIN_PAD, NPAD, CONCAT, NBLK, TPS, FMT, MW, NG, WGS>;
  int rc = get_encoder();
  if (rc) return rc;
  CUtensorMap tm;
  rc = make_tmap(&tm, in_base, (a.a_hi_only ? 1 : 2) * (CIN_PAD / 8), a.N, a.H, a.W, C::HALO_W, C::HALO_H);
  if (rc) return rc;
  a.wpk = wpk;
  a.bias = bias;
  a.in_planes_half = CIN_PAD / 8;
  a.tiles_x = (a.W + C::TILE_W - 1) / C::TILE_W;
  a.tiles_y = (a.H + C::TILE_H - 1) / C::TILE_H;
  const long long tiles = (long long)a.tiles_x * a.tiles_y * a.N * NG;
  auto kern = conv_umma_kernel<KS, CIN_PAD, NPAD, EPI, CONCAT, NBLK, TPS, FMT, RAG, MW, NG, WGS>;
  WN_CUDA(cudaFuncSetAttribute(kern, cudaFuncAttributeMaxDynamicSharedMemorySize, C::SMEM_BYTES));
  TimedScope ts(h, slot, stream);
  const int grid = (int)(tiles < h->sm_count ? tiles : h->sm_count);
  kern<<<grid, C::THREADS, C::SMEM_BYTES, stream>>>(tm, a);
  WN_LAUNCH_CHECK(h);
  return WN_OK;
}

}
```

### waternet_b200/csrc/wgmma_ops.cuh

```cuda
#pragma once

#include <stdint.h>

namespace wn {

template <int N>
__device__ __forceinline__ void wgmma_bf16(float* d, uint64_t da, uint64_t db) {
  if constexpr (N == 16) {
    asm volatile("{\n\t.reg .pred p;\n\tsetp.ne.b32 p, 1, 0;\n\t"
                 "wgmma.mma_async.sync.aligned.m64n16k16.f32.bf16.bf16 {%0, %1, %2, %3, %4, %5, %6, %7}, %8, %9, p, 1, 1, 0, 0;\n\t}"
                 : "+f"(d[0]), "+f"(d[1]), "+f"(d[2]), "+f"(d[3]), "+f"(d[4]), "+f"(d[5]), "+f"(d[6]), "+f"(d[7])
                 : "l"(da), "l"(db));
  } else if constexpr (N == 32) {
    asm volatile("{\n\t.reg .pred p;\n\tsetp.ne.b32 p, 1, 0;\n\t"
                 "wgmma.mma_async.sync.aligned.m64n32k16.f32.bf16.bf16 {%0, %1, %2, %3, %4, %5, %6, %7, %8, %9, %10, %11, %12, %13, %14, %15}, %16, %17, p, 1, 1, 0, 0;\n\t}"
                 : "+f"(d[0]), "+f"(d[1]), "+f"(d[2]), "+f"(d[3]), "+f"(d[4]), "+f"(d[5]), "+f"(d[6]), "+f"(d[7]), "+f"(d[8]), "+f"(d[9]), "+f"(d[10]), "+f"(d[11]), "+f"(d[12]), "+f"(d[13]), "+f"(d[14]), "+f"(d[15])
                 : "l"(da), "l"(db));
  } else if constexpr (N == 64) {
    asm volatile("{\n\t.reg .pred p;\n\tsetp.ne.b32 p, 1, 0;\n\t"
                 "wgmma.mma_async.sync.aligned.m64n64k16.f32.bf16.bf16 {%0, %1, %2, %3, %4, %5, %6, %7, %8, %9, %10, %11, %12, %13, %14, %15, %16, %17, %18, %19, %20, %21, %22, %23, %24, %25, %26, %27, %28, %29, %30, %31}, %32, %33, p, 1, 1, 0, 0;\n\t}"
                 : "+f"(d[0]), "+f"(d[1]), "+f"(d[2]), "+f"(d[3]), "+f"(d[4]), "+f"(d[5]), "+f"(d[6]), "+f"(d[7]), "+f"(d[8]), "+f"(d[9]), "+f"(d[10]), "+f"(d[11]), "+f"(d[12]), "+f"(d[13]), "+f"(d[14]), "+f"(d[15]), "+f"(d[16]), "+f"(d[17]), "+f"(d[18]), "+f"(d[19]), "+f"(d[20]), "+f"(d[21]), "+f"(d[22]), "+f"(d[23]), "+f"(d[24]), "+f"(d[25]), "+f"(d[26]), "+f"(d[27]), "+f"(d[28]), "+f"(d[29]), "+f"(d[30]), "+f"(d[31])
                 : "l"(da), "l"(db));
  } else if constexpr (N == 96) {
    asm volatile("{\n\t.reg .pred p;\n\tsetp.ne.b32 p, 1, 0;\n\t"
                 "wgmma.mma_async.sync.aligned.m64n96k16.f32.bf16.bf16 {%0, %1, %2, %3, %4, %5, %6, %7, %8, %9, %10, %11, %12, %13, %14, %15, %16, %17, %18, %19, %20, %21, %22, %23, %24, %25, %26, %27, %28, %29, %30, %31, %32, %33, %34, %35, %36, %37, %38, %39, %40, %41, %42, %43, %44, %45, %46, %47}, %48, %49, p, 1, 1, 0, 0;\n\t}"
                 : "+f"(d[0]), "+f"(d[1]), "+f"(d[2]), "+f"(d[3]), "+f"(d[4]), "+f"(d[5]), "+f"(d[6]), "+f"(d[7]), "+f"(d[8]), "+f"(d[9]), "+f"(d[10]), "+f"(d[11]), "+f"(d[12]), "+f"(d[13]), "+f"(d[14]), "+f"(d[15]), "+f"(d[16]), "+f"(d[17]), "+f"(d[18]), "+f"(d[19]), "+f"(d[20]), "+f"(d[21]), "+f"(d[22]), "+f"(d[23]), "+f"(d[24]), "+f"(d[25]), "+f"(d[26]), "+f"(d[27]), "+f"(d[28]), "+f"(d[29]), "+f"(d[30]), "+f"(d[31]), "+f"(d[32]), "+f"(d[33]), "+f"(d[34]), "+f"(d[35]), "+f"(d[36]), "+f"(d[37]), "+f"(d[38]), "+f"(d[39]), "+f"(d[40]), "+f"(d[41]), "+f"(d[42]), "+f"(d[43]), "+f"(d[44]), "+f"(d[45]), "+f"(d[46]), "+f"(d[47])
                 : "l"(da), "l"(db));
  } else if constexpr (N == 112) {
    asm volatile("{\n\t.reg .pred p;\n\tsetp.ne.b32 p, 1, 0;\n\t"
                 "wgmma.mma_async.sync.aligned.m64n112k16.f32.bf16.bf16 {%0, %1, %2, %3, %4, %5, %6, %7, %8, %9, %10, %11, %12, %13, %14, %15, %16, %17, %18, %19, %20, %21, %22, %23, %24, %25, %26, %27, %28, %29, %30, %31, %32, %33, %34, %35, %36, %37, %38, %39, %40, %41, %42, %43, %44, %45, %46, %47, %48, %49, %50, %51, %52, %53, %54, %55}, %56, %57, p, 1, 1, 0, 0;\n\t}"
                 : "+f"(d[0]), "+f"(d[1]), "+f"(d[2]), "+f"(d[3]), "+f"(d[4]), "+f"(d[5]), "+f"(d[6]), "+f"(d[7]), "+f"(d[8]), "+f"(d[9]), "+f"(d[10]), "+f"(d[11]), "+f"(d[12]), "+f"(d[13]), "+f"(d[14]), "+f"(d[15]), "+f"(d[16]), "+f"(d[17]), "+f"(d[18]), "+f"(d[19]), "+f"(d[20]), "+f"(d[21]), "+f"(d[22]), "+f"(d[23]), "+f"(d[24]), "+f"(d[25]), "+f"(d[26]), "+f"(d[27]), "+f"(d[28]), "+f"(d[29]), "+f"(d[30]), "+f"(d[31]), "+f"(d[32]), "+f"(d[33]), "+f"(d[34]), "+f"(d[35]), "+f"(d[36]), "+f"(d[37]), "+f"(d[38]), "+f"(d[39]), "+f"(d[40]), "+f"(d[41]), "+f"(d[42]), "+f"(d[43]), "+f"(d[44]), "+f"(d[45]), "+f"(d[46]), "+f"(d[47]), "+f"(d[48]), "+f"(d[49]), "+f"(d[50]), "+f"(d[51]), "+f"(d[52]), "+f"(d[53]), "+f"(d[54]), "+f"(d[55])
                 : "l"(da), "l"(db));
  } else if constexpr (N == 128) {
    asm volatile("{\n\t.reg .pred p;\n\tsetp.ne.b32 p, 1, 0;\n\t"
                 "wgmma.mma_async.sync.aligned.m64n128k16.f32.bf16.bf16 {%0, %1, %2, %3, %4, %5, %6, %7, %8, %9, %10, %11, %12, %13, %14, %15, %16, %17, %18, %19, %20, %21, %22, %23, %24, %25, %26, %27, %28, %29, %30, %31, %32, %33, %34, %35, %36, %37, %38, %39, %40, %41, %42, %43, %44, %45, %46, %47, %48, %49, %50, %51, %52, %53, %54, %55, %56, %57, %58, %59, %60, %61, %62, %63}, %64, %65, p, 1, 1, 0, 0;\n\t}"
                 : "+f"(d[0]), "+f"(d[1]), "+f"(d[2]), "+f"(d[3]), "+f"(d[4]), "+f"(d[5]), "+f"(d[6]), "+f"(d[7]), "+f"(d[8]), "+f"(d[9]), "+f"(d[10]), "+f"(d[11]), "+f"(d[12]), "+f"(d[13]), "+f"(d[14]), "+f"(d[15]), "+f"(d[16]), "+f"(d[17]), "+f"(d[18]), "+f"(d[19]), "+f"(d[20]), "+f"(d[21]), "+f"(d[22]), "+f"(d[23]), "+f"(d[24]), "+f"(d[25]), "+f"(d[26]), "+f"(d[27]), "+f"(d[28]), "+f"(d[29]), "+f"(d[30]), "+f"(d[31]), "+f"(d[32]), "+f"(d[33]), "+f"(d[34]), "+f"(d[35]), "+f"(d[36]), "+f"(d[37]), "+f"(d[38]), "+f"(d[39]), "+f"(d[40]), "+f"(d[41]), "+f"(d[42]), "+f"(d[43]), "+f"(d[44]), "+f"(d[45]), "+f"(d[46]), "+f"(d[47]), "+f"(d[48]), "+f"(d[49]), "+f"(d[50]), "+f"(d[51]), "+f"(d[52]), "+f"(d[53]), "+f"(d[54]), "+f"(d[55]), "+f"(d[56]), "+f"(d[57]), "+f"(d[58]), "+f"(d[59]), "+f"(d[60]), "+f"(d[61]), "+f"(d[62]), "+f"(d[63])
                 : "l"(da), "l"(db));
  } else if constexpr (N == 224) {
    asm volatile("{\n\t.reg .pred p;\n\tsetp.ne.b32 p, 1, 0;\n\t"
                 "wgmma.mma_async.sync.aligned.m64n224k16.f32.bf16.bf16 {%0, %1, %2, %3, %4, %5, %6, %7, %8, %9, %10, %11, %12, %13, %14, %15, %16, %17, %18, %19, %20, %21, %22, %23, %24, %25, %26, %27, %28, %29, %30, %31, %32, %33, %34, %35, %36, %37, %38, %39, %40, %41, %42, %43, %44, %45, %46, %47, %48, %49, %50, %51, %52, %53, %54, %55, %56, %57, %58, %59, %60, %61, %62, %63, %64, %65, %66, %67, %68, %69, %70, %71, %72, %73, %74, %75, %76, %77, %78, %79, %80, %81, %82, %83, %84, %85, %86, %87, %88, %89, %90, %91, %92, %93, %94, %95, %96, %97, %98, %99, %100, %101, %102, %103, %104, %105, %106, %107, %108, %109, %110, %111}, %112, %113, p, 1, 1, 0, 0;\n\t}"
                 : "+f"(d[0]), "+f"(d[1]), "+f"(d[2]), "+f"(d[3]), "+f"(d[4]), "+f"(d[5]), "+f"(d[6]), "+f"(d[7]), "+f"(d[8]), "+f"(d[9]), "+f"(d[10]), "+f"(d[11]), "+f"(d[12]), "+f"(d[13]), "+f"(d[14]), "+f"(d[15]), "+f"(d[16]), "+f"(d[17]), "+f"(d[18]), "+f"(d[19]), "+f"(d[20]), "+f"(d[21]), "+f"(d[22]), "+f"(d[23]), "+f"(d[24]), "+f"(d[25]), "+f"(d[26]), "+f"(d[27]), "+f"(d[28]), "+f"(d[29]), "+f"(d[30]), "+f"(d[31]), "+f"(d[32]), "+f"(d[33]), "+f"(d[34]), "+f"(d[35]), "+f"(d[36]), "+f"(d[37]), "+f"(d[38]), "+f"(d[39]), "+f"(d[40]), "+f"(d[41]), "+f"(d[42]), "+f"(d[43]), "+f"(d[44]), "+f"(d[45]), "+f"(d[46]), "+f"(d[47]), "+f"(d[48]), "+f"(d[49]), "+f"(d[50]), "+f"(d[51]), "+f"(d[52]), "+f"(d[53]), "+f"(d[54]), "+f"(d[55]), "+f"(d[56]), "+f"(d[57]), "+f"(d[58]), "+f"(d[59]), "+f"(d[60]), "+f"(d[61]), "+f"(d[62]), "+f"(d[63]), "+f"(d[64]), "+f"(d[65]), "+f"(d[66]), "+f"(d[67]), "+f"(d[68]), "+f"(d[69]), "+f"(d[70]), "+f"(d[71]), "+f"(d[72]), "+f"(d[73]), "+f"(d[74]), "+f"(d[75]), "+f"(d[76]), "+f"(d[77]), "+f"(d[78]), "+f"(d[79]), "+f"(d[80]), "+f"(d[81]), "+f"(d[82]), "+f"(d[83]), "+f"(d[84]), "+f"(d[85]), "+f"(d[86]), "+f"(d[87]), "+f"(d[88]), "+f"(d[89]), "+f"(d[90]), "+f"(d[91]), "+f"(d[92]), "+f"(d[93]), "+f"(d[94]), "+f"(d[95]), "+f"(d[96]), "+f"(d[97]), "+f"(d[98]), "+f"(d[99]), "+f"(d[100]), "+f"(d[101]), "+f"(d[102]), "+f"(d[103]), "+f"(d[104]), "+f"(d[105]), "+f"(d[106]), "+f"(d[107]), "+f"(d[108]), "+f"(d[109]), "+f"(d[110]), "+f"(d[111])
                 : "l"(da), "l"(db));
  } else {
    static_assert(N < 0, "wgmma shape not generated (tools/gen_wgmma.py)");
  }
}

template <int N>
__device__ __forceinline__ void wgmma_bf16_mn(float* d, uint64_t da, uint64_t db) {
  if constexpr (N == 16) {
    asm volatile("{\n\t.reg .pred p;\n\tsetp.ne.b32 p, 1, 0;\n\t"
                 "wgmma.mma_async.sync.aligned.m64n16k16.f32.bf16.bf16 {%0, %1, %2, %3, %4, %5, %6, %7}, %8, %9, p, 1, 1, 1, 1;\n\t}"
                 : "+f"(d[0]), "+f"(d[1]), "+f"(d[2]), "+f"(d[3]), "+f"(d[4]), "+f"(d[5]), "+f"(d[6]), "+f"(d[7])
                 : "l"(da), "l"(db));
  } else if constexpr (N == 64) {
    asm volatile("{\n\t.reg .pred p;\n\tsetp.ne.b32 p, 1, 0;\n\t"
                 "wgmma.mma_async.sync.aligned.m64n64k16.f32.bf16.bf16 {%0, %1, %2, %3, %4, %5, %6, %7, %8, %9, %10, %11, %12, %13, %14, %15, %16, %17, %18, %19, %20, %21, %22, %23, %24, %25, %26, %27, %28, %29, %30, %31}, %32, %33, p, 1, 1, 1, 1;\n\t}"
                 : "+f"(d[0]), "+f"(d[1]), "+f"(d[2]), "+f"(d[3]), "+f"(d[4]), "+f"(d[5]), "+f"(d[6]), "+f"(d[7]), "+f"(d[8]), "+f"(d[9]), "+f"(d[10]), "+f"(d[11]), "+f"(d[12]), "+f"(d[13]), "+f"(d[14]), "+f"(d[15]), "+f"(d[16]), "+f"(d[17]), "+f"(d[18]), "+f"(d[19]), "+f"(d[20]), "+f"(d[21]), "+f"(d[22]), "+f"(d[23]), "+f"(d[24]), "+f"(d[25]), "+f"(d[26]), "+f"(d[27]), "+f"(d[28]), "+f"(d[29]), "+f"(d[30]), "+f"(d[31])
                 : "l"(da), "l"(db));
  } else if constexpr (N == 96) {
    asm volatile("{\n\t.reg .pred p;\n\tsetp.ne.b32 p, 1, 0;\n\t"
                 "wgmma.mma_async.sync.aligned.m64n96k16.f32.bf16.bf16 {%0, %1, %2, %3, %4, %5, %6, %7, %8, %9, %10, %11, %12, %13, %14, %15, %16, %17, %18, %19, %20, %21, %22, %23, %24, %25, %26, %27, %28, %29, %30, %31, %32, %33, %34, %35, %36, %37, %38, %39, %40, %41, %42, %43, %44, %45, %46, %47}, %48, %49, p, 1, 1, 1, 1;\n\t}"
                 : "+f"(d[0]), "+f"(d[1]), "+f"(d[2]), "+f"(d[3]), "+f"(d[4]), "+f"(d[5]), "+f"(d[6]), "+f"(d[7]), "+f"(d[8]), "+f"(d[9]), "+f"(d[10]), "+f"(d[11]), "+f"(d[12]), "+f"(d[13]), "+f"(d[14]), "+f"(d[15]), "+f"(d[16]), "+f"(d[17]), "+f"(d[18]), "+f"(d[19]), "+f"(d[20]), "+f"(d[21]), "+f"(d[22]), "+f"(d[23]), "+f"(d[24]), "+f"(d[25]), "+f"(d[26]), "+f"(d[27]), "+f"(d[28]), "+f"(d[29]), "+f"(d[30]), "+f"(d[31]), "+f"(d[32]), "+f"(d[33]), "+f"(d[34]), "+f"(d[35]), "+f"(d[36]), "+f"(d[37]), "+f"(d[38]), "+f"(d[39]), "+f"(d[40]), "+f"(d[41]), "+f"(d[42]), "+f"(d[43]), "+f"(d[44]), "+f"(d[45]), "+f"(d[46]), "+f"(d[47])
                 : "l"(da), "l"(db));
  } else if constexpr (N == 128) {
    asm volatile("{\n\t.reg .pred p;\n\tsetp.ne.b32 p, 1, 0;\n\t"
                 "wgmma.mma_async.sync.aligned.m64n128k16.f32.bf16.bf16 {%0, %1, %2, %3, %4, %5, %6, %7, %8, %9, %10, %11, %12, %13, %14, %15, %16, %17, %18, %19, %20, %21, %22, %23, %24, %25, %26, %27, %28, %29, %30, %31, %32, %33, %34, %35, %36, %37, %38, %39, %40, %41, %42, %43, %44, %45, %46, %47, %48, %49, %50, %51, %52, %53, %54, %55, %56, %57, %58, %59, %60, %61, %62, %63}, %64, %65, p, 1, 1, 1, 1;\n\t}"
                 : "+f"(d[0]), "+f"(d[1]), "+f"(d[2]), "+f"(d[3]), "+f"(d[4]), "+f"(d[5]), "+f"(d[6]), "+f"(d[7]), "+f"(d[8]), "+f"(d[9]), "+f"(d[10]), "+f"(d[11]), "+f"(d[12]), "+f"(d[13]), "+f"(d[14]), "+f"(d[15]), "+f"(d[16]), "+f"(d[17]), "+f"(d[18]), "+f"(d[19]), "+f"(d[20]), "+f"(d[21]), "+f"(d[22]), "+f"(d[23]), "+f"(d[24]), "+f"(d[25]), "+f"(d[26]), "+f"(d[27]), "+f"(d[28]), "+f"(d[29]), "+f"(d[30]), "+f"(d[31]), "+f"(d[32]), "+f"(d[33]), "+f"(d[34]), "+f"(d[35]), "+f"(d[36]), "+f"(d[37]), "+f"(d[38]), "+f"(d[39]), "+f"(d[40]), "+f"(d[41]), "+f"(d[42]), "+f"(d[43]), "+f"(d[44]), "+f"(d[45]), "+f"(d[46]), "+f"(d[47]), "+f"(d[48]), "+f"(d[49]), "+f"(d[50]), "+f"(d[51]), "+f"(d[52]), "+f"(d[53]), "+f"(d[54]), "+f"(d[55]), "+f"(d[56]), "+f"(d[57]), "+f"(d[58]), "+f"(d[59]), "+f"(d[60]), "+f"(d[61]), "+f"(d[62]), "+f"(d[63])
                 : "l"(da), "l"(db));
  } else {
    static_assert(N < 0, "wgmma shape not generated (tools/gen_wgmma.py)");
  }
}

template <int N>
__device__ __forceinline__ void wgmma_e4m3(float* d, uint64_t da, uint64_t db) {
  if constexpr (N == 32) {
    asm volatile("{\n\t.reg .pred p;\n\tsetp.ne.b32 p, 1, 0;\n\t"
                 "wgmma.mma_async.sync.aligned.m64n32k32.f32.e4m3.e4m3 {%0, %1, %2, %3, %4, %5, %6, %7, %8, %9, %10, %11, %12, %13, %14, %15}, %16, %17, p, 1, 1;\n\t}"
                 : "+f"(d[0]), "+f"(d[1]), "+f"(d[2]), "+f"(d[3]), "+f"(d[4]), "+f"(d[5]), "+f"(d[6]), "+f"(d[7]), "+f"(d[8]), "+f"(d[9]), "+f"(d[10]), "+f"(d[11]), "+f"(d[12]), "+f"(d[13]), "+f"(d[14]), "+f"(d[15])
                 : "l"(da), "l"(db));
  } else if constexpr (N == 64) {
    asm volatile("{\n\t.reg .pred p;\n\tsetp.ne.b32 p, 1, 0;\n\t"
                 "wgmma.mma_async.sync.aligned.m64n64k32.f32.e4m3.e4m3 {%0, %1, %2, %3, %4, %5, %6, %7, %8, %9, %10, %11, %12, %13, %14, %15, %16, %17, %18, %19, %20, %21, %22, %23, %24, %25, %26, %27, %28, %29, %30, %31}, %32, %33, p, 1, 1;\n\t}"
                 : "+f"(d[0]), "+f"(d[1]), "+f"(d[2]), "+f"(d[3]), "+f"(d[4]), "+f"(d[5]), "+f"(d[6]), "+f"(d[7]), "+f"(d[8]), "+f"(d[9]), "+f"(d[10]), "+f"(d[11]), "+f"(d[12]), "+f"(d[13]), "+f"(d[14]), "+f"(d[15]), "+f"(d[16]), "+f"(d[17]), "+f"(d[18]), "+f"(d[19]), "+f"(d[20]), "+f"(d[21]), "+f"(d[22]), "+f"(d[23]), "+f"(d[24]), "+f"(d[25]), "+f"(d[26]), "+f"(d[27]), "+f"(d[28]), "+f"(d[29]), "+f"(d[30]), "+f"(d[31])
                 : "l"(da), "l"(db));
  } else if constexpr (N == 128) {
    asm volatile("{\n\t.reg .pred p;\n\tsetp.ne.b32 p, 1, 0;\n\t"
                 "wgmma.mma_async.sync.aligned.m64n128k32.f32.e4m3.e4m3 {%0, %1, %2, %3, %4, %5, %6, %7, %8, %9, %10, %11, %12, %13, %14, %15, %16, %17, %18, %19, %20, %21, %22, %23, %24, %25, %26, %27, %28, %29, %30, %31, %32, %33, %34, %35, %36, %37, %38, %39, %40, %41, %42, %43, %44, %45, %46, %47, %48, %49, %50, %51, %52, %53, %54, %55, %56, %57, %58, %59, %60, %61, %62, %63}, %64, %65, p, 1, 1;\n\t}"
                 : "+f"(d[0]), "+f"(d[1]), "+f"(d[2]), "+f"(d[3]), "+f"(d[4]), "+f"(d[5]), "+f"(d[6]), "+f"(d[7]), "+f"(d[8]), "+f"(d[9]), "+f"(d[10]), "+f"(d[11]), "+f"(d[12]), "+f"(d[13]), "+f"(d[14]), "+f"(d[15]), "+f"(d[16]), "+f"(d[17]), "+f"(d[18]), "+f"(d[19]), "+f"(d[20]), "+f"(d[21]), "+f"(d[22]), "+f"(d[23]), "+f"(d[24]), "+f"(d[25]), "+f"(d[26]), "+f"(d[27]), "+f"(d[28]), "+f"(d[29]), "+f"(d[30]), "+f"(d[31]), "+f"(d[32]), "+f"(d[33]), "+f"(d[34]), "+f"(d[35]), "+f"(d[36]), "+f"(d[37]), "+f"(d[38]), "+f"(d[39]), "+f"(d[40]), "+f"(d[41]), "+f"(d[42]), "+f"(d[43]), "+f"(d[44]), "+f"(d[45]), "+f"(d[46]), "+f"(d[47]), "+f"(d[48]), "+f"(d[49]), "+f"(d[50]), "+f"(d[51]), "+f"(d[52]), "+f"(d[53]), "+f"(d[54]), "+f"(d[55]), "+f"(d[56]), "+f"(d[57]), "+f"(d[58]), "+f"(d[59]), "+f"(d[60]), "+f"(d[61]), "+f"(d[62]), "+f"(d[63])
                 : "l"(da), "l"(db));
  } else {
    static_assert(N < 0, "wgmma shape not generated (tools/gen_wgmma.py)");
  }
}

}
```

Baseline: 53.52.

## Use fp8 tap-pair correction path for first layer on exact-integer input slots

Measured after the change: 55.69, median of 6. 4.1% higher.

```diff
diff --git a/waternet_b200/csrc/common.cuh b/waternet_b200/csrc/common.cuh
--- a/waternet_b200/csrc/common.cuh
+++ b/waternet_b200/csrc/common.cuh
@@ -189,6 +189,7 @@
   const TileGeom* tiles = nullptr;
   long long win0 = 0;
   const RaggedWindow* rwin = nullptr;
+  const int* slot_levels = nullptr;
 };
 int umma_forward_layers(wn_handle* h, const float* const in[4], const int64_t st[4][4], float* out, int n,
                         int height, int width, const FwdBuffers& b, cudaStream_t stream,
@@ -240,7 +241,7 @@
 int pack_inputs(wn_handle* h, const GridGeom& geo, const PackInArgs& in, int count, uint4* act0, int* flag,
                 cudaStream_t stream, bool hi = false);
 int pack_inputs(wn_handle* h, const TableGeom& geo, const PackInArgs* imgs, int count, uint4* act0, int* flag,
-                cudaStream_t stream, bool hi = false);
+                cudaStream_t stream, bool hi = false, int* slot_flags = nullptr);
 size_t umma_forward_ragged_workspace_bytes(const int* hs, const int* ws, int n, int tile_h, int tile_w,
                                            long long max_pass_pixels);
 int umma_forward_ragged(wn_handle* h, const wn_ragged_tensors* images, int n, int tile_h, int tile_w,
diff --git a/waternet_b200/csrc/conv_umma.cu b/waternet_b200/csrc/conv_umma.cu
--- a/waternet_b200/csrc/conv_umma.cu
+++ b/waternet_b200/csrc/conv_umma.cu
@@ -41,7 +41,7 @@
   return pack_pixel(imgs[p.img], 0, p.y, p.x, v);
 }
 
-template <class Geom, class In, bool PLANES, bool FLAG, bool HI = false>
+template <class Geom, class In, bool PLANES, bool FLAG, bool HI = false, bool SLOT = false>
 __global__ void __launch_bounds__(256)
 pack_inputs_kernel(Geom geo, In in, uint4* __restrict__ out, int* __restrict__ exact_flag) {
   const int pix = blockIdx.x * 256 + threadIdx.x;
@@ -56,7 +56,7 @@
     if constexpr (PLANES) store_packed<HI>(out + (size_t)blockIdx.y * 4 * hw + pix, hw, v);
   }
   if constexpr (FLAG)
-    if (!__syncthreads_and(exact) && threadIdx.x == 0) atomicExch(exact_flag, 0);
+    if (!__syncthreads_and(exact) && threadIdx.x == 0) atomicExch(exact_flag + (SLOT ? blockIdx.y : 0), 0);
 }
 
 template <bool PLANES, bool FLAG, class Geom, class In>
@@ -79,8 +79,17 @@
   return launch_pack<true, false>(h, geo, in, count, act0, nullptr, false, stream, hi);
 }
 int pack_inputs(wn_handle* h, const TableGeom& geo, const PackInArgs* imgs, int count, uint4* act0, int* flag,
-                cudaStream_t stream, bool hi) {
+                cudaStream_t stream, bool hi, int* slot_flags) {
   if (!act0) return launch_pack<false, true>(h, geo, imgs, count, nullptr, flag, false, stream);
+  if (slot_flags) {
+    TimedScope ts(h, kSlotPack, stream);
+    WN_CUDA(cudaMemsetAsync(slot_flags, 1, (size_t)count * sizeof(int), stream));
+    const dim3 grid((unsigned)(((size_t)geo.slot_hw() + 255) / 256), count);
+    pack_inputs_kernel<TableGeom, const PackInArgs*, true, true, false, true><<<grid, 256, 0, stream>>>(geo, imgs, act0,
+                                                                                                      slot_flags);
+    WN_LAUNCH_CHECK(h);
+    return WN_OK;
+  }
   return launch_pack<true, false>(h, geo, imgs, count, act0, nullptr, false, stream, hi);
 }
 
@@ -128,6 +137,10 @@
 static constexpr int layer_wgs(int li) { return kSpecs[li].wgs; }
 #endif
 
+static constexpr bool pairs_taps(int li) { return li == kL1; }
+static constexpr size_t kPairImageBytes = (size_t)((49 + 1) / 2 + 49) * 224 * 32;
+static constexpr size_t kPairScaleBytes = 2 * 224 * sizeof(float);
+
 static_assert(kSpecs[kC2].f8 == kSpecs[kR2].f8, "L1 writes one format for both of its consumers");
 static constexpr bool writes_f8(int li) { return li < kR3 && li != kC8 && kSpecs[li + 1].f8; }
 
@@ -168,9 +181,11 @@
   for (int i = 0; i < kNumUmmaLayers; i++) {
     if (!h->umma->stages[i]) WN_CUDA(cudaMalloc(&h->umma->stages[i], stage_bytes_total(kSpecs[i])));
     if (!h->umma->bias[i]) WN_CUDA(cudaMalloc(&h->umma->bias[i], kSpecs[i].npad * kSpecs[i].nblk * sizeof(float)));
-    if (kSpecs[i].f8) {
-      if (!h->umma->stages8[i]) WN_CUDA(cudaMalloc(&h->umma->stages8[i], stage_bytes_total(kSpecs[i])));
-      if (!h->umma->scale8[i]) WN_CUDA(cudaMalloc(&h->umma->scale8[i], 4 * sizeof(float)));
+    if (kSpecs[i].f8 || pairs_taps(i)) {
+      const size_t img = pairs_taps(i) ? kPairImageBytes : stage_bytes_total(kSpecs[i]);
+      if (!h->umma->stages8[i]) WN_CUDA(cudaMalloc(&h->umma->stages8[i], img));
+      const size_t sc = pairs_taps(i) ? kPairScaleBytes : 4 * sizeof(float);
+      if (!h->umma->scale8[i]) WN_CUDA(cudaMalloc(&h->umma->scale8[i], sc));
     }
   }
   if (!h->umma->dense) WN_CUDA(cudaMalloc(&h->umma->dense, (size_t)224 * 128 * 49 * sizeof(float)));
@@ -219,6 +234,14 @@
                                                   s.cinpad, kk, s.concat, s.nblk, g * gw);
       WN_LAUNCH_CHECK(h);
     }
+    if (pairs_taps(li)) {
+      static_assert(kSpecs[kL1].cinpad == 16 && kSpecs[kL1].ng == 1 && kSpecs[kL1].nblk == 1 && kSpecs[kL1].npad == 224 &&
+                    kSpecs[kL1].ks == 7, "kPairImageBytes");
+      pair_scale_kernel<<<s.npad, 256, 0, stream>>>(u->dense, u->scale8[li], s.npad, s.cinpad * kk);
+      WN_LAUNCH_CHECK(h);
+      pack_stages_pair_kernel<<<64, 256, 0, stream>>>(u->dense, u->stages8[li], u->scale8[li], s.npad, kk);
+      WN_LAUNCH_CHECK(h);
+    }
     if (s.f8) {
       WN_CUDA(cudaMemsetAsync(u->scale8[li], 0, 4 * sizeof(float), stream));
       f8_absmax_kernel<<<64, 256, 0, stream>>>(u->dense, (size_t)rows * s.cinpad * kk, u->scale8[li]);
@@ -279,9 +302,13 @@
     return launch_conv<s.ks, s.cinpad, GW, s.epi, s.concat, s.nblk, s.tps, kFmtHi, R, s.mw, s.ng, layer_wgs(LI)>(
         h, s.slot, u->stages[LI], u->bias[LI], in_base, a, stream);
   if (scheme == 1) {
-    constexpr int FMT = (s.f8 ? kFmtIn8 : 0) | (writes_f8(LI) ? kFmtOut8 : 0);
+    constexpr int FMT = (s.f8 ? kFmtIn8 : 0) | (writes_f8(LI) ? kFmtOut8 : 0) | (pairs_taps(LI) ? kFmtPair8 : 0);
     if constexpr ((FMT & kFmtOut8) != 0) a.f8_overflow = u->overflow_dev;
     if constexpr (s.f8) a.f8_scale = u->scale8[LI] + 1;
+    if constexpr (pairs_taps(LI)) {
+      a.f8_scale = u->scale8[LI] + s.npad;
+      a.wpk8 = u->stages8[LI];
+    }
     return launch_conv<s.ks, s.cinpad, GW, s.epi, (s.f8 ? 0 : s.concat), s.nblk, s.tps, FMT, R, s.mw, s.ng,
                        layer_wgs(LI)>(h, s.slot, s.f8 ? u->stages8[LI] : u->stages[LI], u->bias[LI], in_base, a, stream);
   }
@@ -376,6 +403,7 @@
   const bool want_cmg = o.stack != kStackRefiners, want_ref = o.stack != kStackCmg;
   a.skip_lo = b.exact_flag;
   a.a_hi_only = o.hi_only ? 1 : 0;
+  a.slot_levels = o.slot_levels;
   if (o.refiner_l1) {
     constexpr UmmaLayerSpec s = kSpecs[kRL1];
     act(b.r[1], 96, nullptr, 0);
@@ -392,6 +420,7 @@
   }
   a.skip_lo = nullptr;
   a.a_hi_only = 0;
+  a.slot_levels = nullptr;
   if (dump(kL1)) return WN_OK;
   if (want_cmg) {
     act(b.a[2], 128, nullptr, 0);
@@ -507,6 +536,8 @@
   if (rc) return rc;
   scheme = effective_scheme(h, scheme);
   const int nb = umma_chunk(h->chunk_pixels, n, H, W);
+  int* flag = nb < n ? carve(workspace, nb, H, W).exact_flag : nullptr;
+  if (flag && (rc = pack_inputs(h, whole_images(H, W), pack_args(in, in_strides), n, nullptr, flag, stream))) return rc;
   for (int n0 = 0; n0 < n; n0 += nb) {
     const int cur = n - n0 < nb ? n - n0 : nb;
     const float* sub[4];
@@ -515,6 +546,13 @@
     FwdOpts o;
     o.scheme = scheme;
     o.stack = stack;
+    if (flag) {
+      b.exact_flag = flag;
+      o.packed = true;
+      if ((rc = pack_inputs(h, whole_images(H, W), pack_args(sub, in_strides), cur, b.act0, nullptr, stream,
+                            scheme == kSchemeBf16)))
+        return rc;
+    }
       float* dst = out + (size_t)n0 * 3 * H * W;
     if (stack == kStackCmg) b.cm = dst;
     if (stack == kStackRefiners) { b.refined = refined + (size_t)n0 * 9 * H * W; dst = nullptr; }
@@ -832,11 +870,13 @@
     FwdBuffers b = carve(fwd_ws, p.count, p.slot_h, p.slot_w);
     b.exact_flag = exact;
     geo.set_pass(p);
-    if ((rc = pack_inputs(h, geo, d_imgs, p.count, b.act0, nullptr, stream))) return rc;
+    int* slot_flags = scheme == 1 ? reinterpret_cast<int*>(b.a[2]) : nullptr;
+    if ((rc = pack_inputs(h, geo, d_imgs, p.count, b.act0, nullptr, stream, false, slot_flags))) return rc;
     FwdOpts o;
     o.scheme = scheme;
     o.packed = true;
     o.rwin = geo.rwin();
+    o.slot_levels = slot_flags;
     rc = umma_pass(h, no_in, none, nullptr, p.count, p.slot_h, p.slot_w, b, stream, o);
     if (rc) return rc;
   }
diff --git a/waternet_b200/csrc/umma_conv.cuh b/waternet_b200/csrc/umma_conv.cuh
--- a/waternet_b200/csrc/umma_conv.cuh
+++ b/waternet_b200/csrc/umma_conv.cuh
@@ -74,13 +74,14 @@
 
 constexpr int kStageLd = 36;
 
-constexpr int kFmtIn8 = 1, kFmtOut8 = 2, kFmtHi = 4;
+constexpr int kFmtIn8 = 1, kFmtOut8 = 2, kFmtHi = 4, kFmtPair8 = 8;
 constexpr int kWgs3ProducerRegs = 24, kWgs3ConsumerRegs = 160;
 template <int KS, int CIN_PAD, int NPAD, int CONCAT = 0, int NBLK = 1, int TPS = 1, int FMT = 0, int MW = 1,
           int NG = 1, int WGS = 2>
 struct UmmaCfg {
   static constexpr bool F8IN = (FMT & kFmtIn8) != 0;
   static constexpr bool HI = (FMT & kFmtHi) != 0;
+  static constexpr bool PAIR = (FMT & kFmtPair8) != 0;
   static constexpr bool DUAL = CONCAT != 0 && !HI;
   static constexpr int TILE_W = 8 * MW, TILE_H = 8 * WGS;
   static constexpr int CONSUMER_WARPS = 4 * WGS;
@@ -95,7 +96,7 @@
   static_assert((KS * KS) % TPS == 0, "taps per weight stage must divide the filter");
   static constexpr int NSTAGE_PER_CHUNK = KS * KS / TPS;
   static constexpr int STAGING = WGS * 64 * kStageLd * 4;
-  static constexpr int BIAS_BYTES = NG * NBLK * NPAD * 4;
+  static constexpr int BIAS_BYTES = NG * NBLK * NPAD * 4 * (PAIR ? 2 : 1);
   static constexpr int TAIL = 512 + (BIAS_BYTES > 1536 ? BIAS_BYTES : 1536);
   static constexpr int BUDGET = 227 * 1024 - 1024 - TAIL - STAGING;
   static constexpr int NA_WANT = NCHUNK == 1 ? 2 : KS == 1 ? 6 : 3;
@@ -105,6 +106,12 @@
   static constexpr int NA = NA_FIT > NA_WANT ? NA_WANT : NA_FIT;
   static_assert(!F8IN || !CONCAT, "fp8 corrections: the [hi | second part] weight layout");
   static_assert(!HI || FMT == kFmtHi, "single-pass bf16 reads and writes bf16 planes only");
+  static_assert(!PAIR || (CIN_PAD == 16 && !CONCAT && NBLK == 1 && TPS == 1 && MW == 1 && NG == 1 && WGS == 2 &&
+                          !F8IN && !HI), "the tap-pair form is the first layer's");
+  static constexpr int PAIRS = (KS * KS + 1) / 2;
+  static constexpr int PAIR_UNITS = PAIRS + KS * KS;
+  static constexpr int PAIR_STAGES = PAIR_UNITS / 2;
+  static_assert(!PAIR || PAIR_UNITS % 2 == 0, "whole weight stages");
   static constexpr int CPB = NCHUNK / NBLK;
   static constexpr int BLK_COLS = DUAL ? 2 * NPAD : NPAD;
   static constexpr int COLS = NBLK * BLK_COLS;
@@ -144,6 +151,8 @@
   const uint4* mask_base;
   int mask_planes_half;
   const float* f8_scale;
+  const uint8_t* wpk8;
+  const int* slot_levels;
   int* f8_overflow;
   const int* run_if;
   int tiled;
@@ -331,7 +340,15 @@
     asm volatile("fence.mbarrier_init.release.cluster;" ::: "memory");
   }
   for (int i = tid; i < NG * NBLK * NPAD; i += C::THREADS) s_bias[i] = g.bias[i];
+  if constexpr (C::PAIR)
+    for (int i = tid; i < NPAD; i += C::THREADS) s_bias[NPAD + i] = g.f8_scale[i];
   __syncthreads();
+  const bool levels = (g.skip_lo != nullptr && *g.skip_lo != 0) || g.a_hi_only;
+  auto pair_tile = [&](int tile) {
+    if (!C::PAIR) return false;
+    if (g.a_hi_only || g.slot_levels == nullptr) return levels;
+    return g.slot_levels[tile / NG / (g.tiles_x * g.tiles_y)] != 0;
+  };
   if constexpr (WGS == 3) {
     if (warp >= C::CONSUMER_WARPS) {
       asm volatile("setmaxnreg.dec.sync.aligned.u32 %0;" ::"n"(kWgs3ProducerRegs));
@@ -366,8 +383,10 @@
       int stage = 0;
       uint32_t phase = 0;
       for (int tile = blockIdx.x; tile < num_tiles; tile += gridDim.x) {
-        const uint8_t* wpk = g.wpk + (size_t)(tile % NG) * C::GROUP_BYTES;
-        for (int it = 0; it < C::NCHUNK * C::NSTAGE_PER_CHUNK; it++) {
+        const bool pair = pair_tile(tile);
+        const uint8_t* wpk = pair ? g.wpk8 : g.wpk + (size_t)(tile % NG) * C::GROUP_BYTES;
+        const int nit = pair ? C::PAIR_STAGES : C::NCHUNK * C::NSTAGE_PER_CHUNK;
+        for (int it = 0; it < nit; it++) {
           mbar_wait(&b_empty[stage], phase ^ 1);
           mbar_expect_tx(&b_full[stage], C::B_STAGE);
           bulk_load(b_stages + stage * C::B_STAGE, wpk + (size_t)it * C::B_STAGE, C::B_STAGE, &b_full[stage]);
@@ -380,7 +399,7 @@
   if constexpr (WGS == 3) asm volatile("setmaxnreg.inc.sync.aligned.u32 %0;" ::"n"(kWgs3ConsumerRegs));
 
   const int wg = warp >> 2, wtid = tid & 127;
-  const bool skip_lo = (g.skip_lo != nullptr && *g.skip_lo != 0) || g.a_hi_only;
+  const bool skip_lo = levels;
   const float dscale0 = F8IN && WGS == 2 ? *g.f8_scale : 1.f;
   constexpr uint32_t kSboA = C::HALO_W * 16;
   constexpr uint32_t kLboB = (CONCAT ? 2 * NPAD : NPAD) * 16;
@@ -395,6 +414,7 @@
     pend_a = pend_b = -1;
   };
   for (int tile = blockIdx.x; tile < num_tiles; tile += gridDim.x) {
+    const bool pair = pair_tile(tile);
 #pragma unroll
     for (int mb = 0; mb < MW; mb++) {
 #pragma unroll
@@ -407,48 +427,101 @@
       mbar_wait(&a_full[astage], aphase);
       const uint32_t a_base = smem_u32(a_stages + astage * C::A_STAGE) + (uint32_t)(wg * 8 * C::HALO_W * 16);
       const int blk = NBLK > 1 ? c / C::CPB : 0;
-      for (int tg = 0; tg < C::NSTAGE_PER_CHUNK; tg++) {
+      if constexpr (C::PAIR) {
+        if (pair) {
+          uint8_t* st = a_stages + astage * C::A_STAGE;
+          for (int p = wtid; p < (8 + KS - 1) * C::HALO_W; p += 128) {
+            const size_t o = (size_t)(wg * 8 * C::HALO_W + p) * 16;
+            const uint4 h0 = *reinterpret_cast<const uint4*>(st + o);
+            const uint4 h1 = *reinterpret_cast<const uint4*>(st + C::PLANE_BYTES + o);
+            const uint32_t hw[8] = {h0.x, h0.y, h0.z, h0.w, h1.x, h1.y, h1.z, h1.w};
+            uint32_t q[4];
+#pragma unroll
+            for (int j = 0; j < 4; j++)
+              q[j] = pack_e4m3x4(__uint_as_float(hw[2 * j] << 16), __uint_as_float(hw[2 * j] & 0xffff0000u),
+                                 __uint_as_float(hw[2 * j + 1] << 16), __uint_as_float(hw[2 * j + 1] & 0xffff0000u));
+            *reinterpret_cast<uint4*>(st + (2 + wg) * C::PLANE_BYTES + o) = make_uint4(q[0], q[1], q[2], q[3]);
+          }
+          asm volatile("fence.proxy.async.shared::cta;" ::: "memory");
+          wg_bar(1 + wg);
+        }
+      }
+      auto stage = [&](bool last_of_chunk, auto&& body) {
         mbar_wait(&b_full[bstage], bphase);
         const uint32_t b_base = smem_u32(b_stages + bstage * C::B_STAGE);
         wg_fence();
-#pragma unroll
-        for (int t = 0; t < TPS; t++) {
-          const int tap = tg * TPS + t;
-          const int ky = tap / KS, kx = tap - ky * KS;
-          const uint32_t a_tap = a_base + (uint32_t)((ky * C::HALO_W + kx) * 16);
-          const uint32_t b_tap = b_base + (uint32_t)(t * C::B_TAP);
-          const uint64_t a_hi0 = make_desc(a_tap, C::PLANE_BYTES, kSboA);
-#pragma unroll
-          for (int mb = 0; mb < MW; mb++) {
-            const uint64_t a_hi = a_hi0 + mb * (128 >> 4);
-            const uint64_t a_lo = MW == 1 ? make_desc(a_tap + 2 * C::PLANE_BYTES, C::PLANE_BYTES, kSboA)
-                                          : a_hi + ((2 * C::PLANE_BYTES) >> 4);
-#pragma unroll
-            for (int b = 0; b < NBLK; b++) {
-              if (NBLK > 1 && b != blk) continue;
-              float* d = acc[mb] + b * C::BLK_COLS / 2;
-              if constexpr (C::HI) {
-                wgmma_bf16<NPAD>(d, a_hi, make_desc(b_tap, kLboB, 128));
-              } else if constexpr (F8IN) {
-                wgmma_bf16<NPAD>(d, a_hi, make_desc(b_tap, NPAD * 16, 128));
-                wgmma_e4m3<NPAD>(acc8[mb] + b * C::BLK_COLS / 2, a_lo, make_desc(b_tap + NPAD * 32, NPAD * 16, 128));
-              } else if constexpr (CONCAT) {
-                wgmma_bf16<2 * NPAD>(d, a_hi, make_desc(b_tap, kLboB, 128));
-                if (!skip_lo) wgmma_bf16<NPAD>(d, a_lo, make_desc(b_tap, kLboB, 128));
-              } else {
-                wgmma_bf16<NPAD>(d, a_hi, make_desc(b_tap, kLboB, 128));
-                if (!skip_lo) wgmma_bf16<NPAD>(d, a_lo, make_desc(b_tap, kLboB, 128));
-                wgmma_bf16<NPAD>(d, a_hi, make_desc(b_tap + 2 * NPAD * 16, kLboB, 128));
-              }
-            }
-          }
-        }
+        body(b_base);
         wg_commit();
         wg_wait<1>();
         release();
         pend_b = bstage;
-        if (tg == C::NSTAGE_PER_CHUNK - 1) pend_a = astage;
+        if (last_of_chunk) pend_a = astage;
         if (++bstage == C::NB) { bstage = 0; bphase ^= 1; }
+      };
+      bool issued = false;
+      if constexpr (C::PAIR) {
+        if (pair) {
+#pragma unroll
+          for (int tg = 0; tg < C::PAIR_STAGES; tg++) {
+            stage(tg == C::PAIR_STAGES - 1, [&](uint32_t b_base) {
+#pragma unroll
+              for (int j = 0; j < 2; j++) {
+                const int u = 2 * tg + j;
+                const uint32_t b_unit = b_base + (uint32_t)(j * NPAD * 32);
+                if (u < C::PAIRS) {
+                  const int t0 = 2 * u < KS * KS - 2 ? 2 * u : KS * KS - 2, t1 = t0 + 1;
+                  const uint32_t o0 = (uint32_t)(((t0 / KS) * C::HALO_W + t0 % KS) * 16);
+                  const uint32_t o1 = (uint32_t)(((t1 / KS) * C::HALO_W + t1 % KS) * 16);
+                  const uint32_t a_pair = a_base + (2 + wg) * C::PLANE_BYTES + o0;
+                  wgmma_e4m3<C::PAIR ? NPAD : 32>(acc[0], make_desc(a_pair, o1 - o0, kSboA), make_desc(b_unit, NPAD * 16, 128));
+                } else {
+                  const int tap = u - C::PAIRS;
+                  const uint32_t a_tap = a_base + (uint32_t)(((tap / KS) * C::HALO_W + tap % KS) * 16);
+                  wgmma_bf16<NPAD>(acc[0], make_desc(a_tap, C::PLANE_BYTES, kSboA), make_desc(b_unit, NPAD * 16, 128));
+                }
+              }
+            });
+          }
+          issued = true;
+        }
+      }
+      if (!issued) {
+        for (int tg = 0; tg < C::NSTAGE_PER_CHUNK; tg++) {
+          stage(tg == C::NSTAGE_PER_CHUNK - 1, [&](uint32_t b_base) {
+#pragma unroll
+            for (int t = 0; t < TPS; t++) {
+              const int tap = tg * TPS + t;
+              const int ky = tap / KS, kx = tap - ky * KS;
+              const uint32_t a_tap = a_base + (uint32_t)((ky * C::HALO_W + kx) * 16);
+              const uint32_t b_tap = b_base + (uint32_t)(t * C::B_TAP);
+              const uint64_t a_hi0 = make_desc(a_tap, C::PLANE_BYTES, kSboA);
+#pragma unroll
+              for (int mb = 0; mb < MW; mb++) {
+                const uint64_t a_hi = a_hi0 + mb * (128 >> 4);
+                const uint64_t a_lo = MW == 1 ? make_desc(a_tap + 2 * C::PLANE_BYTES, C::PLANE_BYTES, kSboA)
+                                              : a_hi + ((2 * C::PLANE_BYTES) >> 4);
+#pragma unroll
+                for (int b = 0; b < NBLK; b++) {
+                  if (NBLK > 1 && b != blk) continue;
+                  float* d = acc[mb] + b * C::BLK_COLS / 2;
+                  if constexpr (C::HI) {
+                    wgmma_bf16<NPAD>(d, a_hi, make_desc(b_tap, kLboB, 128));
+                  } else if constexpr (F8IN) {
+                    wgmma_bf16<NPAD>(d, a_hi, make_desc(b_tap, NPAD * 16, 128));
+                    wgmma_e4m3<NPAD>(acc8[mb] + b * C::BLK_COLS / 2, a_lo, make_desc(b_tap + NPAD * 32, NPAD * 16, 128));
+                  } else if constexpr (CONCAT) {
+                    wgmma_bf16<2 * NPAD>(d, a_hi, make_desc(b_tap, kLboB, 128));
+                    if (!skip_lo) wgmma_bf16<NPAD>(d, a_lo, make_desc(b_tap, kLboB, 128));
+                  } else {
+                    wgmma_bf16<NPAD>(d, a_hi, make_desc(b_tap, kLboB, 128));
+                    if (!skip_lo) wgmma_bf16<NPAD>(d, a_lo, make_desc(b_tap, kLboB, 128));
+                    wgmma_bf16<NPAD>(d, a_hi, make_desc(b_tap + 2 * NPAD * 16, kLboB, 128));
+                  }
+                }
+              }
+            }
+          });
+        }
       }
       if (++astage == C::NA) { astage = 0; aphase ^= 1; }
     }
@@ -485,6 +558,7 @@
               v[k] = acc[mb][col / 2 + k];
               if constexpr (DUAL) v[k] += acc[mb][(col + NPAD) / 2 + k];
               if constexpr (F8IN) v[k] = (v[k] + acc8[mb][col / 2 + k]) * dscale;
+              if constexpr (C::PAIR) v[k] = pair ? v[k] * s_bias[NPAD + col + fcol + (k & 1)] : v[k];
             }
             float* s = stg + frow * kStageLd + 8 * j + fcol;
             *reinterpret_cast<float2*>(s) = make_float2(v[0], v[1]);
@@ -606,6 +680,57 @@
     *reinterpret_cast<uint16_t*>(p1 + ((size_t)0 * rows + row) * 16 + c) = pack_e4m3x2(w[0] * ws, w[1] * ws);
     *reinterpret_cast<uint16_t*>(p1 + ((size_t)1 * rows + row) * 16 + c) =
         pack_e4m3x2(wl[0] * ws * 512.f, wl[1] * ws * 512.f);
+  }
+}
+
+static __global__ void pair_scale_kernel(const float* __restrict__ dense, float* __restrict__ scale, int npad, int n) {
+  __shared__ float smax[256];
+  float m = 0.f;
+  for (int i = threadIdx.x; i < n; i += blockDim.x) m = fmaxf(m, fabsf(dense[(size_t)blockIdx.x * n + i]));
+  smax[threadIdx.x] = m;
+  __syncthreads();
+  for (int o = 128; o > 0; o >>= 1) {
+    if ((int)threadIdx.x < o) smax[threadIdx.x] = fmaxf(smax[threadIdx.x], smax[threadIdx.x + o]);
+    __syncthreads();
+  }
+  if (threadIdx.x == 0) {
+    const float s = exp2f(floorf(log2f(224.f / fmaxf(smax[0], 1e-30f))));
+    scale[blockIdx.x] = s;
+    scale[npad + blockIdx.x] = 1.f / (512.f * s);
+  }
+}
+static __global__ void pack_stages_pair_kernel(const float* __restrict__ dense, uint8_t* __restrict__ out,
+                                               const float* __restrict__ scale, int npad, int kk) {
+  const int pairs = (kk + 1) / 2, units = pairs + kk;
+  for (int i = blockIdx.x * blockDim.x + threadIdx.x; i < units * npad; i += gridDim.x * blockDim.x) {
+    const int u = i / npad, row = i - u * npad;
+    const float s = scale[row] * 512.f;
+    uint8_t* unit = out + (size_t)u * npad * 32;
+    const float* w = dense + (size_t)row * 16 * kk;
+    if (u < pairs) {
+      const int t0 = 2 * u < kk - 2 ? 2 * u : kk - 2;
+      for (int h = 0; h < 2; h++) {
+        const int tap = t0 + h;
+        const bool zero = h == 0 && 2 * u >= kk - 1;
+        uint32_t q[4];
+        for (int j = 0; j < 4; j++) {
+          float f[4];
+          for (int e = 0; e < 4; e++) {
+            const float x = w[(4 * j + e) * kk + tap];
+            f[e] = zero ? 0.f : (x - __bfloat162float(__float2bfloat16_rn(x))) * s;
+          }
+          q[j] = pack_e4m3x4(f[0], f[1], f[2], f[3]);
+        }
+        *reinterpret_cast<uint4*>(unit + ((size_t)h * npad + row) * 16) = make_uint4(q[0], q[1], q[2], q[3]);
+      }
+    } else {
+      const int tap = u - pairs;
+      for (int c = 0; c < 16; c++) {
+        const float hi = __bfloat162float(__float2bfloat16_rn(w[c * kk + tap])) * s;
+        *reinterpret_cast<__nv_bfloat16*>(unit + ((size_t)(c / 8) * npad + row) * 16 + (c % 8) * 2) =
+            __float2bfloat16_rn(hi);
+      }
+    }
   }
 }
 
diff --git a/waternet_b200/csrc/wgmma_ops.cuh b/waternet_b200/csrc/wgmma_ops.cuh
--- a/waternet_b200/csrc/wgmma_ops.cuh
+++ b/waternet_b200/csrc/wgmma_ops.cuh
@@ -90,6 +90,11 @@
                  "wgmma.mma_async.sync.aligned.m64n128k32.f32.e4m3.e4m3 {%0, %1, %2, %3, %4, %5, %6, %7, %8, %9, %10, %11, %12, %13, %14, %15, %16, %17, %18, %19, %20, %21, %22, %23, %24, %25, %26, %27, %28, %29, %30, %31, %32, %33, %34, %35, %36, %37, %38, %39, %40, %41, %42, %43, %44, %45, %46, %47, %48, %49, %50, %51, %52, %53, %54, %55, %56, %57, %58, %59, %60, %61, %62, %63}, %64, %65, p, 1, 1;\n\t}"
                  : "+f"(d[0]), "+f"(d[1]), "+f"(d[2]), "+f"(d[3]), "+f"(d[4]), "+f"(d[5]), "+f"(d[6]), "+f"(d[7]), "+f"(d[8]), "+f"(d[9]), "+f"(d[10]), "+f"(d[11]), "+f"(d[12]), "+f"(d[13]), "+f"(d[14]), "+f"(d[15]), "+f"(d[16]), "+f"(d[17]), "+f"(d[18]), "+f"(d[19]), "+f"(d[20]), "+f"(d[21]), "+f"(d[22]), "+f"(d[23]), "+f"(d[24]), "+f"(d[25]), "+f"(d[26]), "+f"(d[27]), "+f"(d[28]), "+f"(d[29]), "+f"(d[30]), "+f"(d[31]), "+f"(d[32]), "+f"(d[33]), "+f"(d[34]), "+f"(d[35]), "+f"(d[36]), "+f"(d[37]), "+f"(d[38]), "+f"(d[39]), "+f"(d[40]), "+f"(d[41]), "+f"(d[42]), "+f"(d[43]), "+f"(d[44]), "+f"(d[45]), "+f"(d[46]), "+f"(d[47]), "+f"(d[48]), "+f"(d[49]), "+f"(d[50]), "+f"(d[51]), "+f"(d[52]), "+f"(d[53]), "+f"(d[54]), "+f"(d[55]), "+f"(d[56]), "+f"(d[57]), "+f"(d[58]), "+f"(d[59]), "+f"(d[60]), "+f"(d[61]), "+f"(d[62]), "+f"(d[63])
                  : "l"(da), "l"(db));
+  } else if constexpr (N == 224) {
+    asm volatile("{\n\t.reg .pred p;\n\tsetp.ne.b32 p, 1, 0;\n\t"
+                 "wgmma.mma_async.sync.aligned.m64n224k32.f32.e4m3.e4m3 {%0, %1, %2, %3, %4, %5, %6, %7, %8, %9, %10, %11, %12, %13, %14, %15, %16, %17, %18, %19, %20, %21, %22, %23, %24, %25, %26, %27, %28, %29, %30, %31, %32, %33, %34, %35, %36, %37, %38, %39, %40, %41, %42, %43, %44, %45, %46, %47, %48, %49, %50, %51, %52, %53, %54, %55, %56, %57, %58, %59, %60, %61, %62, %63, %64, %65, %66, %67, %68, %69, %70, %71, %72, %73, %74, %75, %76, %77, %78, %79, %80, %81, %82, %83, %84, %85, %86, %87, %88, %89, %90, %91, %92, %93, %94, %95, %96, %97, %98, %99, %100, %101, %102, %103, %104, %105, %106, %107, %108, %109, %110, %111}, %112, %113, p, 1, 1;\n\t}"
+                 : "+f"(d[0]), "+f"(d[1]), "+f"(d[2]), "+f"(d[3]), "+f"(d[4]), "+f"(d[5]), "+f"(d[6]), "+f"(d[7]), "+f"(d[8]), "+f"(d[9]), "+f"(d[10]), "+f"(d[11]), "+f"(d[12]), "+f"(d[13]), "+f"(d[14]), "+f"(d[15]), "+f"(d[16]), "+f"(d[17]), "+f"(d[18]), "+f"(d[19]), "+f"(d[20]), "+f"(d[21]), "+f"(d[22]), "+f"(d[23]), "+f"(d[24]), "+f"(d[25]), "+f"(d[26]), "+f"(d[27]), "+f"(d[28]), "+f"(d[29]), "+f"(d[30]), "+f"(d[31]), "+f"(d[32]), "+f"(d[33]), "+f"(d[34]), "+f"(d[35]), "+f"(d[36]), "+f"(d[37]), "+f"(d[38]), "+f"(d[39]), "+f"(d[40]), "+f"(d[41]), "+f"(d[42]), "+f"(d[43]), "+f"(d[44]), "+f"(d[45]), "+f"(d[46]), "+f"(d[47]), "+f"(d[48]), "+f"(d[49]), "+f"(d[50]), "+f"(d[51]), "+f"(d[52]), "+f"(d[53]), "+f"(d[54]), "+f"(d[55]), "+f"(d[56]), "+f"(d[57]), "+f"(d[58]), "+f"(d[59]), "+f"(d[60]), "+f"(d[61]), "+f"(d[62]), "+f"(d[63]), "+f"(d[64]), "+f"(d[65]), "+f"(d[66]), "+f"(d[67]), "+f"(d[68]), "+f"(d[69]), "+f"(d[70]), "+f"(d[71]), "+f"(d[72]), "+f"(d[73]), "+f"(d[74]), "+f"(d[75]), "+f"(d[76]), "+f"(d[77]), "+f"(d[78]), "+f"(d[79]), "+f"(d[80]), "+f"(d[81]), "+f"(d[82]), "+f"(d[83]), "+f"(d[84]), "+f"(d[85]), "+f"(d[86]), "+f"(d[87]), "+f"(d[88]), "+f"(d[89]), "+f"(d[90]), "+f"(d[91]), "+f"(d[92]), "+f"(d[93]), "+f"(d[94]), "+f"(d[95]), "+f"(d[96]), "+f"(d[97]), "+f"(d[98]), "+f"(d[99]), "+f"(d[100]), "+f"(d[101]), "+f"(d[102]), "+f"(d[103]), "+f"(d[104]), "+f"(d[105]), "+f"(d[106]), "+f"(d[107]), "+f"(d[108]), "+f"(d[109]), "+f"(d[110]), "+f"(d[111])
+                 : "l"(da), "l"(db));
   } else {
     static_assert(N < 0, "wgmma shape not generated (tools/gen_wgmma.py)");
   }
```
